# hkchengrex/Cutie

Measured on AMD Instinct MI355X. Metric: frames/sec (480p, 3 objects), higher is better.
Workload: dtype bf16

## Files before the change

cutie_amd/_lib.py:

```python
import ctypes
import os

_HERE = os.path.dirname(os.path.abspath(__file__))
LIB_PATH = os.environ.get('CUTIE_AMD_LIB') or os.path.join(_HERE, 'libcutie_hip.so')
ABI_VERSION = 11
OP_STRUCT_SIZE = 256

_lib = None


class HipLibraryError(RuntimeError):
    pass


def load():
    global _lib
    if _lib is not None:
        return _lib
    if not os.path.exists(LIB_PATH):
        raise HipLibraryError(
            f'{LIB_PATH} not found: build it with `python -c "import __graft_entry__ as g; g.build()"` '
            f'(or `make -C cutie_amd/csrc`).  cutie_amd has no CPU fallback.')
    lib = ctypes.CDLL(LIB_PATH)
    lib.cutie_exec.argtypes = [ctypes.c_void_p, ctypes.c_int, ctypes.c_void_p]
    lib.cutie_exec.restype = ctypes.c_int
    lib.cutie_exec_one.argtypes = [ctypes.c_void_p, ctypes.c_void_p]
    lib.cutie_exec_one.restype = ctypes.c_int
    lib.cutie_graph_capture.argtypes = [ctypes.c_void_p, ctypes.c_int, ctypes.c_void_p]
    lib.cutie_graph_capture.restype = ctypes.c_void_p
    lib.cutie_graph_launch.argtypes = [ctypes.c_void_p, ctypes.c_void_p]
    lib.cutie_graph_launch.restype = ctypes.c_int
    lib.cutie_graph_destroy.argtypes = [ctypes.c_void_p]
    lib.cutie_graph_destroy.restype = None
    lib.cutie_time_ops.argtypes = [ctypes.c_void_p, ctypes.c_int, ctypes.c_int, ctypes.c_void_p]
    lib.cutie_time_ops.restype = ctypes.c_float
    lib.cutie_hip_last_error.argtypes = []
    lib.cutie_hip_last_error.restype = ctypes.c_char_p
    lib.cutie_hip_abi_version.restype = ctypes.c_int
    lib.cutie_op_struct_size.restype = ctypes.c_int
    lib.cutie_hip_build_flags.restype = ctypes.c_int
    if lib.cutie_hip_abi_version() != ABI_VERSION or lib.cutie_op_struct_size() != OP_STRUCT_SIZE:
        raise HipLibraryError(f'{LIB_PATH} is stale (ABI {lib.cutie_hip_abi_version()}, '
                              f'op size {lib.cutie_op_struct_size()}); rebuild it.')
    _lib = lib
    return lib


EXPORTED_SYMBOLS = ['cutie_exec', 'cutie_exec_one', 'cutie_graph_capture', 'cutie_graph_launch',
                    'cutie_graph_destroy', 'cutie_time_ops', 'cutie_hip_last_error',
                    'cutie_hip_abi_version', 'cutie_op_struct_size', 'cutie_hip_build_flags']


def has_diag_kernels():
    return bool(load().cutie_hip_build_flags() & 1)


def has_png_decode():
    return bool(load().cutie_hip_build_flags() & 2)


def has_jpeg_batch():
    return bool(load().cutie_hip_build_flags() & 4)


def has_mixed_lockstep():
    return bool(load().cutie_hip_build_flags() & 8)


def has_track_stats():
    return bool(load().cutie_hip_build_flags() & 16)


class HipExecutor:
    is_mock = False

    def __init__(self):
        import torch
        self.lib = load()
        if not torch.cuda.is_available():
            raise HipLibraryError('no HIP device visible: cutie_amd runs on MI355X only (no CPU fallback).')
        self._torch = torch
        self._raw_stream = getattr(torch._C, '_cuda_getCurrentRawStream', None)
        self.graph_stats = [0, 0]
        self._warned = False

    def stream(self):
        raw = self._raw_stream
        if raw is not None:
            return raw(self._torch.cuda.current_device())
        return self._torch.cuda.current_stream().cuda_stream

    def run(self, arr):
        rc = self.lib.cutie_exec(arr.ctypes.data, len(arr), self.stream())
        if rc != 0:
            raise RuntimeError('cutie_exec failed: ' + self.lib.cutie_hip_last_error().decode())

    def run_on(self, arr, stream):
        rc = self.lib.cutie_exec(arr.ctypes.data, len(arr), stream.cuda_stream)
        if rc != 0:
            raise RuntimeError('cutie_exec failed: ' + self.lib.cutie_hip_last_error().decode())

    GRAPH_CACHE_ENTRIES = 24

    def run_cached(self, arr, cache, head=0):
        if head:
            self.run(arr[:head])
            arr = arr[head:]
        key = arr['p'].tobytes()
        ent = cache.get(key)
        if ent is None:
            if len(cache) >= self.GRAPH_CACHE_ENTRIES:
                old = cache.pop(next(iter(cache)))
                if old not in (0, -1):
                    self.lib.cutie_graph_destroy(old)
            cache[key] = 0
            self.graph_stats[0] += 1
            return self.run(arr)
        if ent == 0:
            ent = self.lib.cutie_graph_capture(arr.ctypes.data, len(arr), self.stream()) or -1
            cache[key] = ent
            if ent == -1 and not self._warned:
                self._warned = True
                import warnings
                warnings.warn('HIP graph capture of a launch plan failed (%s); such plans keep running launch by launch'
                              % self.lib.cutie_hip_last_error().decode())
        if ent == -1:
            self.graph_stats[0] += 1
            return self.run(arr)
        self.graph_stats[1] += 1
        if self.lib.cutie_graph_launch(ent, self.stream()) != 0:
            raise RuntimeError('cutie_graph_launch failed: ' + self.lib.cutie_hip_last_error().decode())

    def time_ops(self, arr, iters):
        ms = self.lib.cutie_time_ops(arr.ctypes.data, len(arr), iters, self.stream())
        if ms < 0:
            raise RuntimeError('cutie_time_ops failed: ' + self.lib.cutie_hip_last_error().decode())
        return ms


_executor = None


def get_executor():
    global _executor
    if _executor is None:
        _executor = HipExecutor()
    return _executor


def set_executor_for_testing(ex):
    global _executor
    _executor = ex
```

cutie_amd/csrc/api.hip:

```cpp
#include "common.h"
#include <stdarg.h>
#include <stdio.h>
#include <string.h>

static thread_local char g_err[512] = "";

void cutie_set_error(const char* fmt, ...) {
    va_list ap;
    va_start(ap, fmt);
    vsnprintf(g_err, sizeof(g_err), fmt, ap);
    va_end(ap);
}

static int dispatch(const cutie_op* op, hipStream_t s) {
    switch (op->kind) {
        case CUTIE_OP_CONV: return launch_conv(op, s);
        case CUTIE_OP_QUERY_INIT: return (op->flags & 1) ? launch_attention(op, s) : launch_elementwise(op, s);
        case CUTIE_OP_QFFN: return launch_qchain(op, s);
        case CUTIE_OP_STEM: return launch_stem(op, s);
        case CUTIE_OP_ATTN_Q2P: case CUTIE_OP_ATTN_SELF: case CUTIE_OP_ATTN_P2Q:
            return (op->flags & 12) ? launch_qchain(op, s) : launch_attention(op, s);
        case CUTIE_OP_AUX_MASK:
            return launch_attention(op, s);
        case CUTIE_OP_KEY_PREP: case CUTIE_OP_AFF_SCORE: case CUTIE_OP_AFF_SELECT: case CUTIE_OP_AFF_READOUT:
// ... 21 lines not shown
                cutie_set_error("op %d (kind %d): %s", k, ops[k].kind, tmp);
            }
            return rc > 0 ? -1 : rc;
        }
    }
    return 0;
}

int cutie_exec_one(const cutie_op* op, void* stream) { return cutie_exec(op, 1, stream); }

struct GraphHandle { hipGraph_t graph; hipGraphExec_t exec; };

void* cutie_graph_capture(const cutie_op* ops, int n, void* stream) {
    (void)stream;
    static thread_local hipStream_t cap = nullptr;
    if (!cap && hipStreamCreateWithFlags(&cap, hipStreamNonBlocking) != hipSuccess) {
        cap = nullptr;
        (void)hipGetLastError();
        cutie_set_error("graph: cannot create the capture stream");
        return nullptr;
    }
    hipGraph_t graph = nullptr;
    if (hipStreamBeginCapture(cap, hipStreamCaptureModeThreadLocal) != hipSuccess) {
        (void)hipGetLastError();
        cutie_set_error("graph: begin capture failed");
        return nullptr;
    }
    int rc = cutie_exec(ops, n, (void*)cap);
    hipError_t e = hipStreamEndCapture(cap, &graph);
    if (rc != 0 || e != hipSuccess || !graph) {
        if (graph) hipGraphDestroy(graph);
        if (rc == 0) cutie_set_error("graph: end capture failed (%d)", (int)e);
        (void)hipGetLastError();
        return nullptr;
    }
    hipGraphExec_t exec = nullptr;
    if (hipGraphInstantiate(&exec, graph, nullptr, nullptr, 0) != hipSuccess) {
        hipGraphDestroy(graph);
        (void)hipGetLastError();
        cutie_set_error("graph: instantiate failed");
        return nullptr;
    }
    GraphHandle* h = new GraphHandle{graph, exec};
    return h;
}

int cutie_graph_launch(void* graph, void* stream) {
    GraphHandle* h = (GraphHandle*)graph;
    if (!h) { cutie_set_error("graph: null handle"); return -4; }
    hipError_t e = hipGraphLaunch(h->exec, (hipStream_t)stream);
    if (e != hipSuccess) { cutie_set_error("graph launch: %s", hipGetErrorString(e)); return -1; }
    return 0;
}

void cutie_graph_destroy(void* graph) {
    GraphHandle* h = (GraphHandle*)graph;
    if (!h) return;
    hipGraphExecDestroy(h->exec);
    hipGraphDestroy(h->graph);
    delete h;
}

float cutie_time_ops(const cutie_op* ops, int n, int iters, void* stream) {
    hipStream_t s = (hipStream_t)stream;
    hipEvent_t a, b;
    if (hipEventCreate(&a) != hipSuccess || hipEventCreate(&b) != hipSuccess) { cutie_set_error("time: event create failed"); return -1.f; }
    if (cutie_exec(ops, n, stream) != 0) return -1.f;
    hipEventRecord(a, s);
    for (int it = 0; it < iters; ++it)
        if (cutie_exec(ops, n, stream) != 0) return -1.f;
    hipEventRecord(b, s);
    hipEventSynchronize(b);
    float ms = 0.f;
    hipEventElapsedTime(&ms, a, b);
    hipEventDestroy(a);
    hipEventDestroy(b);
    return ms / (float)iters;
}

const char* cutie_hip_last_error(void) { return g_err; }
int cutie_hip_abi_version(void) { return 11; }
int cutie_op_struct_size(void) { return (int)sizeof(cutie_op); }
int cutie_hip_build_flags(void) {
    const int forms = 2 | 4 | 8 | 16;
#ifdef CUTIE_DIAG
    return forms | 1;
#else
    return forms;
#endif
}

}
```

cutie_amd/csrc/elementwise.hip:

```cpp
#include "common.h"
#include <math.h>

#define GRID1D(n, bs) dim3((unsigned)(((long)(n) + (bs) - 1) / (bs)))
__global__ void memset32_kernel(uint32_t* d, long n, uint32_t v);

__global__ void maxpool_kernel(const uint4* __restrict__ x, uint4* __restrict__ y, int B, int H, int W, int C8,
                               int OH, int OW, int relu) {
    long idx = (long)blockIdx.x * blockDim.x + threadIdx.x;
    long total = (long)B * OH * OW * C8;
    if (idx >= total) return;
    int c = idx % C8; long t = idx / C8;
    int ow = t % OW; t /= OW; int oh = t % OH; int b = t / OH;
    float m[8];
#pragma unroll
    for (int i = 0; i < 8; ++i) m[i] = relu ? 0.f : -INFINITY;
    for (int dy = 0; dy < 3; ++dy) {
        int ih = oh * 2 - 1 + dy;
        if ((unsigned)ih >= (unsigned)H) continue;
        for (int dx = 0; dx < 3; ++dx) {
            int iw = ow * 2 - 1 + dx;
            if ((unsigned)iw >= (unsigned)W) continue;
            uint4 v = x[(((long)b * H + ih) * W + iw) * C8 + c];
            uint32_t u[4] = {v.x, v.y, v.z, v.w};
#pragma unroll
            for (int i = 0; i < 4; ++i) {
                m[2 * i] = fmaxf(m[2 * i], __uint_as_float(u[i] << 16));
                m[2 * i + 1] = fmaxf(m[2 * i + 1], __uint_as_float(u[i] & 0xffff0000u));
            }
        }
    }
    y[idx] = make_uint4(pack_bf2(m[0], m[1]), pack_bf2(m[2], m[3]), pack_bf2(m[4], m[5]), pack_bf2(m[6], m[7]));
}

__global__ void img_prep_kernel(const float* __restrict__ img, const float* __restrict__ masks, uint4* __restrict__ y,
                                int h0, int w0, int H, int W, int pl, int pt, int K,
                                float m0, float m1, float m2, float s0, float s1, float s2) {
    long idx = (long)blockIdx.x * blockDim.x + threadIdx.x;
    long HW = (long)H * W;
    if (idx >= HW * K) return;
    int k = idx / HW; long pix = idx - (long)k * HW;
    int yy = pix / W, xx = pix - (long)yy * W;
    int sy = yy - pt, sx = xx - pl;
    float r = 0.f, g = 0.f, b = 0.f;
    if ((unsigned)sy < (unsigned)h0 && (unsigned)sx < (unsigned)w0) {
        long o = (long)sy * w0 + sx, plane = (long)h0 * w0;
        r = img[o]; g = img[plane + o]; b = img[2 * plane + o];
    }
    r = (r - m0) / s0; g = (g - m1) / s1; b = (b - m2) / s2;
    float mk = 0.f, others = 0.f;
    if (masks) {
        float sum = 0.f;
        for (int j = 0; j < K; ++j) sum += masks[(long)j * HW + pix];
        mk = masks[(long)k * HW + pix];
        others = fminf(fmaxf(sum - mk, 0.f), 1.f);
    }
    y[idx] = make_uint4(pack_bf2(r, g), pack_bf2(b, mk), pack_bf2(others, 0.f), 0u);
}

__device__ __forceinline__ void up_coord(int o, int n_in, float scale, int& i0, int& i1, float& lam) {
    float src = ((float)o + 0.5f) * scale - 0.5f;
    if (src < 0.f) src = 0.f;
    i0 = (int)src;
    if (i0 > n_in - 1) i0 = n_in - 1;
    i1 = i0 + (i0 < n_in - 1 ? 1 : 0);
    lam = src - (float)i0;
}

template <bool MIXED = false>
__global__ void upsample2x_add_kernel(const uint4* __restrict__ g, const uint4* __restrict__ skip, uint4* __restrict__ y,
                                      int B, int h, int w, int C8, int Kg, long gstride, int prio) {
    if (prio) __builtin_amdgcn_s_setprio(1);
    long idx = (long)blockIdx.x * blockDim.x + threadIdx.x;
    int OH = 2 * h, OW = 2 * w;
    long total = (long)B * OH * OW * C8;
    if (idx >= total) return;
    int c = idx % C8; long t = idx / C8;
    int ox = t % OW; t /= OW; int oy = t % OH; int b = t / OH;
    int y0, y1, x0, x1; float ly, lx;
    up_coord(oy, h, 0.5f, y0, y1, ly);
    up_coord(ox, w, 0.5f, x0, x1, lx);
    const uint4* gb = g + (long)b * h * w * C8;
    uint4 v00 = gb[((long)y0 * w + x0) * C8 + c], v01 = gb[((long)y0 * w + x1) * C8 + c];
    uint4 v10 = gb[((long)y1 * w + x0) * C8 + c], v11 = gb[((long)y1 * w + x1) * C8 + c];
    long grp;
    if (MIXED) { int st; grp = mixed_clip_of((unsigned)Kg, b, st); }
    else grp = Kg > 0 ? b / Kg : 0;
    uint4 sk = skip[(grp * gstride + (long)oy * OW + ox) * C8 + c];
    const uint32_t* a = &v00.x; const uint32_t* bq = &v01.x; const uint32_t* cq = &v10.x; const uint32_t* d = &v11.x;
    const uint32_t* s = &sk.x;
    float w00 = (1.f - ly) * (1.f - lx), w01 = (1.f - ly) * lx, w10 = ly * (1.f - lx), w11 = ly * lx;
    uint32_t out[4];
#pragma unroll
    for (int i = 0; i < 4; ++i) {
        float lo = w00 * __uint_as_float(a[i] << 16) + w01 * __uint_as_float(bq[i] << 16) +
                   w10 * __uint_as_float(cq[i] << 16) + w11 * __uint_as_float(d[i] << 16) + __uint_as_float(s[i] << 16);
        float hi = w00 * __uint_as_float(a[i] & 0xffff0000u) + w01 * __uint_as_float(bq[i] & 0xffff0000u) +
                   w10 * __uint_as_float(cq[i] & 0xffff0000u) + w11 * __uint_as_float(d[i] & 0xffff0000u) +
                   __uint_as_float(s[i] & 0xffff0000u);
        out[i] = pack_bf2(lo, hi);
    }
    y[idx] = make_uint4(out[0], out[1], out[2], out[3]);
}

template <int R = 0>
__device__ __forceinline__ void area_down_bf16_body(const bf16_t* __restrict__ x, bf16_t* __restrict__ y, int B, int H, int W, int C,
                                                    int ldx, int ldy, int rrt, long idx) {
    const int r = R > 0 ? R : rrt;
    int C8 = C >> 3, OH = H / r, OW = W / r;
    long total = (long)B * OH * OW * C8;
    if (idx >= total) return;
    int c = idx % C8; long t = idx / C8;
    int ox = t % OW; t /= OW; int oy = t % OH; int b = t / OH;
    float acc[8] = {0, 0, 0, 0, 0, 0, 0, 0};
    if (R > 0) {
        uint4 v[R > 0 ? R * R : 1];
#pragma unroll
        for (int dy = 0; dy < R; ++dy)
#pragma unroll
            for (int dx = 0; dx < R; ++dx)
                v[dy * R + dx] = *reinterpret_cast<const uint4*>(x + (((long)b * H + oy * R + dy) * W + ox * R + dx) * ldx + c * 8);
#pragma unroll
        for (int e = 0; e < R * R; ++e) {
            const uint32_t* u = &v[e].x;
#pragma unroll
            for (int i = 0; i < 4; ++i) {
                acc[2 * i] += __uint_as_float(u[i] << 16);
                acc[2 * i + 1] += __uint_as_float(u[i] & 0xffff0000u);
            }
        }
    } else
    for (int dy = 0; dy < r; ++dy)
        for (int dx = 0; dx < r; ++dx) {
            const uint4 v = *reinterpret_cast<const uint4*>(x + (((long)b * H + oy * r + dy) * W + ox * r + dx) * ldx + c * 8);
            const uint32_t* u = &v.x;
#pragma unroll
            for (int i = 0; i < 4; ++i) {
                acc[2 * i] += __uint_as_float(u[i] << 16);
                acc[2 * i + 1] += __uint_as_float(u[i] & 0xffff0000u);
            }
        }
    float inv = 1.f / (float)(r * r);
    uint4 o = make_uint4(pack_bf2(acc[0] * inv, acc[1] * inv), pack_bf2(acc[2] * inv, acc[3] * inv),
                         pack_bf2(acc[4] * inv, acc[5] * inv), pack_bf2(acc[6] * inv, acc[7] * inv));
    *reinterpret_cast<uint4*>(y + (((long)b * OH + oy) * OW + ox) * ldy + c * 8) = o;
}
__global__ void area_down_bf16_kernel(const bf16_t* __restrict__ x, bf16_t* __restrict__ y, int B, int H, int W, int C,
                                      int ldx, int ldy, int r) {
    area_down_bf16_body(x, y, B, H, W, C, ldx, ldy, r, (long)blockIdx.x * blockDim.x + threadIdx.x);
}

template <int R = 0>
__device__ __forceinline__ void area_down_f32_body(const float* __restrict__ x, bf16_t* __restrict__ y, int B, int H, int W, int C,
                                                   int ldx, int ldy, int rrt, int Cz, long idx) {
    const int r = R > 0 ? R : rrt;
    int OH = H / r, OW = W / r;
    long total = (long)B * OH * OW;
    if (idx >= total) return;
    int ox = idx % OW; long t = idx / OW; int oy = t % OH; int b = t / OH;
    float inv = 1.f / (float)(r * r);
    bf16_t* yp = y + idx * ldy;
    for (int c = 0; c < C; ++c) {
        float acc = 0.f;
        if (R > 0) {
            float v[R > 0 ? R * R : 1];
#pragma unroll
            for (int dy = 0; dy < R; ++dy)
#pragma unroll
                for (int dx = 0; dx < R; ++dx) v[dy * R + dx] = x[(((long)b * H + oy * R + dy) * W + ox * R + dx) * ldx + c];
#pragma unroll
            for (int e = 0; e < R * R; ++e) acc += v[e];
        } else
        for (int dy = 0; dy < r; ++dy)
            for (int dx = 0; dx < r; ++dx) acc += x[(((long)b * H + oy * r + dy) * W + ox * r + dx) * ldx + c];
        yp[c] = f2bf(acc * inv);
    }
    for (int c = C; c < Cz; ++c) yp[c] = 0;
}
__global__ void area_down_f32_kernel(const float* __restrict__ x, bf16_t* __restrict__ y, int B, int H, int W, int C,
                                     int ldx, int ldy, int r, int Cz) {
    area_down_f32_body(x, y, B, H, W, C, ldx, ldy, r, Cz, (long)blockIdx.x * blockDim.x + threadIdx.x);
}
struct AreaSeg { const void* x; bf16_t* y; int B, H, W, C, ldx, ldy, r, Cz, f32; long n; };
struct Area3 { AreaSeg s[3]; int rt; int prio; };
__global__ void area_down3_kernel(Area3 a) {
// ... 57 lines not shown
            if (k0 + u >= K) break;
            const float a = wave_sum(acc[u]) / (float)(r * r);
            sum += a;
            if (lane == 0) m16[(long)(k0 + u) * hw + px] = a;
        }
    }
    if (lane == 0)
        for (int k = 0; k < K; ++k) {
            const float mk = m16[(long)k * hw + px];
            const float others = fminf(fmaxf(sum - mk, 0.f), 1.f);
            y[((long)k * hw + px) * ld8] = make_uint4(pack_bf2(mk, others), 0u, 0u, 0u);
        }
}
__global__ void mask_pair_kernel(const float* __restrict__ m16, uint4* __restrict__ y, int K, int hw) {
    long idx = (long)blockIdx.x * blockDim.x + threadIdx.x;
    if (idx >= (long)K * hw) return;
    int k = idx / hw; int p = idx - (long)k * hw;
    float sum = 0.f;
    for (int j = 0; j < K; ++j) sum += m16[(long)j * hw + p];
    float mk = m16[idx];
    float others = fminf(fmaxf(sum - mk, 0.f), 1.f);
    y[idx] = make_uint4(pack_bf2(mk, others), 0u, 0u, 0u);
}

__global__ __launch_bounds__(256) void gap_partial_kernel(const bf16_t* __restrict__ x, float* __restrict__ part, int HW, int C) {
    __shared__ float red[2048 + 32];
    const int b = blockIdx.y, p0 = blockIdx.x * 64;
    const int C8 = C >> 3;
    const int c8 = threadIdx.x % C8, rg = threadIdx.x / C8, nrg = 256 / C8;
    float acc[8] = {0, 0, 0, 0, 0, 0, 0, 0};
    for (int r = rg; r < 64; r += nrg) {
        int p = p0 + r;
        if (p < HW) {
            uint4 v = *reinterpret_cast<const uint4*>(x + ((long)b * HW + p) * C + c8 * 8);
            acc[0] += __uint_as_float(v.x << 16); acc[1] += __uint_as_float(v.x & 0xffff0000u);
            acc[2] += __uint_as_float(v.y << 16); acc[3] += __uint_as_float(v.y & 0xffff0000u);
            acc[4] += __uint_as_float(v.z << 16); acc[5] += __uint_as_float(v.z & 0xffff0000u);
            acc[6] += __uint_as_float(v.w << 16); acc[7] += __uint_as_float(v.w & 0xffff0000u);
        }
    }
#pragma unroll
    for (int i = 0; i < 8; ++i) red[rg * (C + 1) + c8 * 8 + i] = acc[i];
    __syncthreads();
    for (int c = threadIdx.x; c < C; c += 256) {
        float sum = 0.f;
        for (int g = 0; g < nrg; ++g) sum += red[g * (C + 1) + c];
        part[((long)b * gridDim.x + blockIdx.x) * C + c] = sum;
    }
}
__global__ void gap_final_kernel(const float* __restrict__ part, float* __restrict__ y, int nchunk, int C, float inv) {
    const int b = blockIdx.x;
    for (int c = threadIdx.x; c < C; c += blockDim.x) {
        float sum = 0.f;
        for (int k = 0; k < nchunk; ++k) sum += part[((long)b * nchunk + k) * C + c];
        y[(long)b * C + c] = sum * inv;
    }
}

__global__ __launch_bounds__(256) void eca_apply_kernel(const bf16_t* __restrict__ x, const float* __restrict__ part,
                                                        const float* __restrict__ wk, const bf16_t* __restrict__ r,
                                                        bf16_t* __restrict__ y, float* __restrict__ gap_out, int HW, int C, int nchunk,
                                                        const long long* __restrict__ fixed, const bf16_t* __restrict__ pw,
                                                        const float* __restrict__ pb, float* __restrict__ plog, int prio) {
    if (prio) __builtin_amdgcn_s_setprio(1);
    __shared__ float gap[256 + 4], sc[256];
    const int b = blockIdx.y, tid = threadIdx.x;
    const float inv = 1.f / (float)HW;
    const int C8 = C >> 3;
    const int p0 = blockIdx.x * 32;
    uint4 xv[4], rv[4];
    long offs[4];
#pragma unroll
    for (int it = 0; it < 4; ++it) {
        const int q = tid + it * 256;
        const int pp = q / C8, c8 = q - pp * C8, p = p0 + pp;
        const bool ok = q < 32 * C8 && p < HW;
        offs[it] = ok ? ((long)b * HW + p) * C + c8 * 8 : -1;
        const long o = ok ? offs[it] : 0;
        xv[it] = *reinterpret_cast<const uint4*>(x + o);
        rv[it] = *reinterpret_cast<const uint4*>(r + o);
    }
    if (fixed) {
        for (int c = tid; c < C; c += 256) {
            const float mean = (float)((double)fixed[(long)b * C + c] * (1.0 / 16777216.0)) * inv;
            gap[c + 2] = mean;
            if (gap_out && blockIdx.x == 0) gap_out[(long)b * C + c] = mean;
        }
    } else
    for (int c = tid; c < C; c += 256) {
        float sum = 0.f;
        for (int k0 = 0; k0 < nchunk; k0 += 8) {
            float v[8];
#pragma unroll
            for (int u = 0; u < 8; ++u) v[u] = part[((long)b * nchunk + min(k0 + u, nchunk - 1)) * C + c];
#pragma unroll
            for (int u = 0; u < 8; ++u) sum += k0 + u < nchunk ? v[u] : 0.f;
        }
        gap[c + 2] = sum * inv;
        if (gap_out && blockIdx.x == 0) gap_out[(long)b * C + c] = sum * inv;
    }
    if (tid < 2) { gap[tid] = 0.f; gap[C + 2 + tid] = 0.f; }
    __syncthreads();
    for (int c = tid; c < C; c += 256) {
        float a = wk[0] * gap[c] + wk[1] * gap[c + 1] + wk[2] * gap[c + 2] + wk[3] * gap[c + 3] + wk[4] * gap[c + 4];
        sc[(c & 7) * 32 + (c >> 3)] = sigmoidf_(a);
    }
    __syncthreads();
#pragma unroll
    for (int it = 0; it < 4; ++it) {
        if (offs[it] < 0) continue;
        const int q = tid + it * 256;
        const int c8 = q % C8;
        const uint32_t* xu = &xv[it].x; const uint32_t* ru = &rv[it].x;
        uint32_t o[4];
#pragma unroll
        for (int i = 0; i < 4; ++i) {
            float lo = __uint_as_float(xu[i] << 16) * sc[(2 * i) * 32 + c8] + __uint_as_float(ru[i] << 16);
            float hi = __uint_as_float(xu[i] & 0xffff0000u) * sc[(2 * i + 1) * 32 + c8] + __uint_as_float(ru[i] & 0xffff0000u);
            o[i] = pack_bf2(lo, hi);
        }
        *reinterpret_cast<uint4*>(y + offs[it]) = make_uint4(o[0], o[1], o[2], o[3]);
    }
    if (pw) {
        const int c8 = tid & 31;
        const uint4 wv = *reinterpret_cast<const uint4*>(pw + c8 * 8);
        const uint32_t* wu = &wv.x;
        const float bias = pb ? pb[0] : 0.f;
#pragma unroll
        for (int it = 0; it < 4; ++it) {
            float part = 0.f;
            if (offs[it] >= 0) {
                const uint32_t* xu = &xv[it].x; const uint32_t* ru = &rv[it].x;
#pragma unroll
                for (int i = 0; i < 4; ++i) {
                    const float lo = __uint_as_float(xu[i] << 16) * sc[(2 * i) * 32 + c8] + __uint_as_float(ru[i] << 16);
                    const float hi = __uint_as_float(xu[i] & 0xffff0000u) * sc[(2 * i + 1) * 32 + c8] + __uint_as_float(ru[i] & 0xffff0000u);
                    const uint32_t st = pack_bf2(lo, hi);
                    part += fmaxf(__uint_as_float(st << 16), 0.f) * __uint_as_float(wu[i] << 16);
                    part += fmaxf(__uint_as_float(st & 0xffff0000u), 0.f) * __uint_as_float(wu[i] & 0xffff0000u);
                }
            }
            part += __uint_as_float(__builtin_amdgcn_update_dpp(0, (int)__float_as_uint(part), 0xB1, 0xf, 0xf, false));
            part += __uint_as_float(__builtin_amdgcn_update_dpp(0, (int)__float_as_uint(part), 0x4E, 0xf, 0xf, false));
            part += __uint_as_float(__builtin_amdgcn_update_dpp(0, (int)__float_as_uint(part), 0x141, 0xf, 0xf, false));
            part += __uint_as_float(__builtin_amdgcn_update_dpp(0, (int)__float_as_uint(part), 0x140, 0xf, 0xf, false));
            const unsigned pu = __float_as_uint(part);
            const auto rr = __builtin_amdgcn_permlane16_swap(pu, pu, false, false);
            const float tot = __uint_as_float(rr[0]) + __uint_as_float(rr[1]);
            const int q = tid + it * 256, p = p0 + q / C8;
            if (c8 == 0 && offs[it] >= 0) plog[(long)b * HW + p] = tot + bias;
        }
    }
}

__global__ void gru4_kernel(const float* __restrict__ v, float* __restrict__ h, bf16_t* __restrict__ hb, long n, int C, int prio) {
    if (prio) __builtin_amdgcn_s_setprio(1);
    const long idx = (long)blockIdx.x * blockDim.x + threadIdx.x;
    const int C4 = C >> 2;
    if (idx >= n * C4) return;
    const long row = idx / C4; const int c = (int)(idx - row * C4) * 4;
    const float* vr = v + row * 3 * C + c;
    const float4 f4 = *reinterpret_cast<const float4*>(vr), u4 = *reinterpret_cast<const float4*>(vr + C), n4 = *reinterpret_cast<const float4*>(vr + 2 * C);
    const float4 h4 = *reinterpret_cast<const float4*>(h + row * C + c);
    const float fa[4] = {f4.x, f4.y, f4.z, f4.w}, ua[4] = {u4.x, u4.y, u4.z, u4.w}, na[4] = {n4.x, n4.y, n4.z, n4.w}, ha[4] = {h4.x, h4.y, h4.z, h4.w};
    float o[4];
#pragma unroll
    for (int i = 0; i < 4; ++i) {
        const float f = sigmoidf_(fa[i]), u = sigmoidf_(ua[i]), nv = tanhf(na[i]);
        o[i] = f * ha[i] * (1.f - u) + u * nv;
    }
    *reinterpret_cast<float4*>(h + row * C + c) = make_float4(o[0], o[1], o[2], o[3]);
    *reinterpret_cast<uint2*>(hb + row * C + c) = make_uint2(pack_bf2(o[0], o[1]), pack_bf2(o[2], o[3]));
}

__global__ void gru_kernel(const float* __restrict__ v, float* __restrict__ h, bf16_t* __restrict__ hb, long n, int C) {
    long idx = (long)blockIdx.x * blockDim.x + threadIdx.x;
    if (idx >= n * C) return;
    long row = idx / C; int c = idx - row * C;
    const float* vr = v + row * 3 * C;
    float f = sigmoidf_(vr[c]), u = sigmoidf_(vr[C + c]), nv = tanhf(vr[2 * C + c]);
    float nh = f * h[idx] * (1.f - u) + u * nv;
    h[idx] = nh;
    hb[idx] = f2bf(nh);
}

__device__ __forceinline__ float clamp_logit(float p) {
    p = fminf(fmaxf(p, 1e-7f), 1.f - 1e-7f);
    return logf(p / (1.f - p));
}

__global__ void seg_agg_kernel(const float* __restrict__ lg, float* __restrict__ agg, int K, int hw) {
    int p = blockIdx.x * blockDim.x + threadIdx.x;
    if (p >= hw) return;
    float bg = 1.f;
    for (int k = 0; k < K; ++k) {
        float pr = 1.f / (1.f + expf(-lg[(long)k * hw + p]));
        bg *= (1.f - pr);
        agg[(long)(k + 1) * hw + p] = clamp_logit(pr);
    }
    agg[p] = clamp_logit(bg);
}

__global__ void up4_softmax_kernel(const float* __restrict__ agg, float* __restrict__ prob, float* __restrict__ lup,
                                   int P, int h, int w) {
    int OH = 4 * h, OW = 4 * w;
    long idx = (long)blockIdx.x * blockDim.x + threadIdx.x;
    if (idx >= (long)OH * OW) return;
    int ox = idx % OW, oy = idx / OW;
    int y0, y1, x0, x1; float ly, lx;
    up_coord(oy, h, 0.25f, y0, y1, ly);
    up_coord(ox, w, 0.25f, x0, x1, lx);
    float w00 = (1.f - ly) * (1.f - lx), w01 = (1.f - ly) * lx, w10 = ly * (1.f - lx), w11 = ly * lx;
    long o00 = (long)y0 * w + x0, o01 = (long)y0 * w + x1, o10 = (long)y1 * w + x0, o11 = (long)y1 * w + x1;
    long hw = (long)h * w, OHW = (long)OH * OW;
    float mx = -INFINITY;
    for (int c = 0; c < P; ++c) {
        const float* a = agg + c * hw;
        float v = w00 * a[o00] + w01 * a[o01] + w10 * a[o10] + w11 * a[o11];
        if (lup) lup[c * OHW + idx] = v;
        mx = fmaxf(mx, v);
    }
    float sum = 0.f;
    for (int c = 0; c < P; ++c) {
        const float* a = agg + c * hw;
        float v = w00 * a[o00] + w01 * a[o01] + w10 * a[o10] + w11 * a[o11];
        sum += expf(v - mx);
    }
    float inv = 1.f / sum;
    for (int c = 0; c < P; ++c) {
        const float* a = agg + c * hw;
        float v = w00 * a[o00] + w01 * a[o01] + w10 * a[o10] + w11 * a[o11];
// ... 807 lines not shown
#pragma unroll
    for (int k = 0; k < 4; ++k)
        if (ox0 + k < OW) o[k] = (OUT)lut[arg[k]];
}

template <typename OUT>
__global__ void prob_to_id_merge_kernel(const uint64_t* __restrict__ srcs, const int4* __restrict__ geom, const int* __restrict__ lut,
                                        OUT* __restrict__ out, int S, int P, int OH, int OW, int packed) {
    const int OW4 = (OW + 3) >> 2;
    const long idx = (long)blockIdx.x * blockDim.x + threadIdx.x;
    if (idx >= (long)OH * OW4) return;
    const int oy = (int)(idx / OW4), ox0 = (int)(idx - (long)oy * OW4) * 4;
    int best[4], arg[4];
#pragma unroll
    for (int k = 0; k < 4; ++k) { best[k] = 0; arg[k] = 0; }
    for (int q = 0; q < P; ++q) {
        int sum[4] = {0, 0, 0, 0};
        for (int sI = 0; sI < S; ++sI) {
            const int4 g = geom[sI];
            const int H = g.x, W = g.y;
            if (H < 1 || W < 1) continue;
            const float* prob = (const float*)srcs[sI] + (long)q * g.z;
            const float sy = (float)H / (float)OH, sx = (float)W / (float)OW;
            const float fy = fmaxf((oy + 0.5f) * sy - 0.5f, 0.f);
            const int y0 = min((int)fy, H - 1), y1 = min(y0 + 1, H - 1);
            const float ly = fy - (float)y0;
            const float* r0 = prob + (long)y0 * g.w;
            const float* r1 = prob + (long)y1 * g.w;
#pragma unroll
            for (int k = 0; k < 4; ++k) {
                const int ox = min(ox0 + k, OW - 1);
                const float fx = fmaxf((ox + 0.5f) * sx - 0.5f, 0.f);
                const int x0 = min((int)fx, W - 1), x1 = min(x0 + 1, W - 1);
                const float lx = fx - (float)x0;
                const float a = r0[x0], b = r0[x1], cc = r1[x0], d = r1[x1];
                const float v = (1.f - ly) * ((1.f - lx) * a + lx * b) + ly * ((1.f - lx) * cc + lx * d);
                sum[k] += (int)(uint8_t)(int)(v * 255.f);
            }
        }
#pragma unroll
        for (int k = 0; k < 4; ++k)
            if (q == 0 || sum[k] > best[k]) { best[k] = sum[k]; arg[k] = q; }
    }
    OUT* o = out + (long)oy * OW + ox0;
    if constexpr (sizeof(OUT) == 1) {
        if (packed) {
            *(uint32_t*)o = (uint32_t)(uint8_t)lut[arg[0]] | (uint32_t)(uint8_t)lut[arg[1]] << 8 | (uint32_t)(uint8_t)lut[arg[2]] << 16 |
                            (uint32_t)(uint8_t)lut[arg[3]] << 24;
            return;
        }
    } else {
        if (packed) {
            *(int4*)o = make_int4(lut[arg[0]], lut[arg[1]], lut[arg[2]], lut[arg[3]]);
            return;
        }
    }
#pragma unroll
    for (int k = 0; k < 4; ++k)
        if (ox0 + k < OW) o[k] = (OUT)lut[arg[k]];
}

int launch_elementwise(const cutie_op* op, hipStream_t s) {
    const int32_t* i = op->i;
    const uint64_t* p = op->p;
    const int BS = 256;
    const int PRIO = (op->flags & CUTIE_F_PRIO) ? 1 : 0;
    switch (op->kind) {
        case CUTIE_OP_MAXPOOL: {
            int C8 = i[3] / 8;
            long n = (long)i[0] * i[4] * i[5] * C8;
            hipLaunchKernelGGL(maxpool_kernel, GRID1D(n, BS), dim3(BS), 0, s, (const uint4*)p[0], (uint4*)p[1], i[0], i[1], i[2], C8, i[4], i[5], op->flags & 1);
            break;
        }
        case CUTIE_OP_IMG_PREP: {
            int K = p[1] ? i[6] : 1;
            long n = (long)i[2] * i[3] * K;
            hipLaunchKernelGGL(img_prep_kernel, GRID1D(n, BS), dim3(BS), 0, s, (const float*)p[0], (const float*)p[1], (uint4*)p[2],
                               i[0], i[1], i[2], i[3], i[4], i[5], K, op->f[0], op->f[1], op->f[2], op->f[3], op->f[4], op->f[5]);
            break;
        }
        case CUTIE_OP_UPSAMPLE2X_ADD: {
            int C8 = i[3] / 8;
            long n = (long)i[0] * 4 * i[1] * i[2] * C8;
            if (i[6]) {
                int objs; const int nc = mixed_clips((unsigned)i[6], &objs);
                if (nc < 1 || objs != i[0] || i[4] != 0 || i[5] < 4 * i[1] * i[2]) { cutie_set_error("upsample2x_add (mixed form): the counts 0x%x do not add up to B = %d (or i4 != 0, or the stride is below one map)", i[6], i[0]); return -2; }
                hipLaunchKernelGGL(upsample2x_add_kernel<true>, GRID1D(n, BS), dim3(BS), 0, s, (const uint4*)p[0], (const uint4*)p[1], (uint4*)p[2], i[0], i[1], i[2], C8, i[6], (long)i[5], PRIO);
                break;
            }
            if (i[4] < 0 || (i[4] > 0 && (i[0] % i[4] || i[5] < 4 * i[1] * i[2]))) { cutie_set_error("upsample2x_add: skip groups of %d objects do not divide B = %d (or their stride is below one map)", i[4], i[0]); return -2; }
            hipLaunchKernelGGL(upsample2x_add_kernel<false>, GRID1D(n, BS), dim3(BS), 0, s, (const uint4*)p[0], (const uint4*)p[1], (uint4*)p[2], i[0], i[1], i[2], C8, i[4], (long)i[5], PRIO);
            break;
        }
        case CUTIE_OP_AREA_DOWN: {
            int r = i[6];
            long np = (long)i[0] * (i[1] / r) * (i[2] / r);
            if (op->flags & 1)
                hipLaunchKernelGGL(area_down_f32_kernel, GRID1D(np, BS), dim3(BS), 0, s, (const float*)p[0], (bf16_t*)p[1], i[0], i[1], i[2], i[3], i[4], i[5], r, i[7]);
            else
                hipLaunchKernelGGL(area_down_bf16_kernel, GRID1D(np * (i[3] / 8), BS), dim3(BS), 0, s, (const bf16_t*)p[0], (bf16_t*)p[1], i[0], i[1], i[2], i[3], i[4], i[5], r);
            break;
        }
        case CUTIE_OP_AREA_DOWN3: {
            Area3 a;
            long total = 0;
            for (int q = 0; q < 3; ++q) {
                const int32_t* j = i + 8 * q;
                AreaSeg& g = a.s[q];
                g.x = (const void*)p[2 * q]; g.y = (bf16_t*)p[2 * q + 1];
                g.B = j[0]; g.H = j[1]; g.W = j[2]; g.C = j[3]; g.ldx = j[4]; g.ldy = j[5]; g.r = j[6]; g.Cz = j[7];
                g.f32 = (op->flags >> q) & 1;
                if (g.r < 1 || (!g.f32 && (g.C & 7))) { cutie_set_error("area_down3: segment %d: r >= 1, C %% 8 for bf16 input", q); return -2; }
                const long np = (long)g.B * (g.H / g.r) * (g.W / g.r);
                g.n = g.f32 ? np : np * (g.C / 8);
                total += g.n;
            }
            a.rt = (op->flags >> 3) & 1;
            a.prio = PRIO;
            hipLaunchKernelGGL(area_down3_kernel, GRID1D(total, BS), dim3(BS), 0, s, a);
            break;
        }
        case CUTIE_OP_MASK_DOWN: {
            int K = i[0], r = i[3], h = i[1] / r, w = i[2] / r;
            long n = (long)K * h * w;
            float* m16 = (float*)p[2];
            if (!m16) { cutie_set_error("mask_down: m16 buffer required"); return -2; }
            hipLaunchKernelGGL(mask_down_pair_kernel, GRID1D((long)h * w * 64, BS), dim3(BS), 0, s, (const float*)p[0], m16, (uint4*)p[1], K, i[1], i[2], r,
                               i[4] > 8 ? i[4] / 8 : 1);
            break;
        }
        case CUTIE_OP_GAP: {
            if (i[2] > 256 || (i[2] & 7) || 256 % (i[2] / 8)) { cutie_set_error("gap: C must divide 256 octet-wise (C=%d)", i[2]); return -2; }
            if (!p[2]) { cutie_set_error("gap: scratch buffer required"); return -2; }
            int nchunk = (i[1] + 63) / 64;
            hipLaunchKernelGGL(gap_partial_kernel, dim3(nchunk, i[0]), dim3(256), 0, s, (const bf16_t*)p[0], (float*)p[2], i[1], i[2]);
            if (!(op->flags & 1))
                hipLaunchKernelGGL(gap_final_kernel, dim3(i[0]), dim3(256), 0, s, (const float*)p[2], (float*)p[1], nchunk, i[2], 1.f / (float)i[1]);
            break;
        }
        case CUTIE_OP_ECA_APPLY: {
            if (i[2] > 256 || (i[2] & 7)) { cutie_set_error("eca: C <= 256, C %% 8"); return -2; }
            if (p[6] && (i[2] != 256 || !p[8])) { cutie_set_error("eca: the fused 1x1 head needs C = 256 and an output"); return -2; }
            int nchunk = (i[1] + 63) / 64;
            hipLaunchKernelGGL(eca_apply_kernel, dim3((i[1] + 31) / 32, i[0]), dim3(256), 0, s, (const bf16_t*)p[0], (const float*)p[5], (const float*)p[2],
                               (const bf16_t*)p[3], (bf16_t*)p[4], (float*)p[1], i[1], i[2], nchunk, (op->flags & 1) ? (const long long*)p[5] : nullptr,
                               (const bf16_t*)p[6], (const float*)p[7], (float*)p[8], PRIO);
            break;
        }
        case CUTIE_OP_GRU: {
            long n = (long)i[0] * i[1];
            if (!(op->flags & 1) && (i[1] & 3) == 0 && (((uintptr_t)p[0] | (uintptr_t)p[1]) & 15) == 0 && ((uintptr_t)p[2] & 7) == 0)
                hipLaunchKernelGGL(gru4_kernel, GRID1D(n / 4, BS), dim3(BS), 0, s, (const float*)p[0], (float*)p[1], (bf16_t*)p[2], (long)i[0], i[1], PRIO);
            else
                hipLaunchKernelGGL(gru_kernel, GRID1D(n, BS), dim3(BS), 0, s, (const float*)p[0], (float*)p[1], (bf16_t*)p[2], (long)i[0], i[1]);
            break;
        }
        case CUTIE_OP_SEG_AGG:
            hipLaunchKernelGGL(seg_agg_kernel, GRID1D(i[1], BS), dim3(BS), 0, s, (const float*)p[0], (float*)p[1], i[0], i[1]);
            break;
        case CUTIE_OP_UP4_SOFTMAX: {
            long n = (long)16 * i[1] * i[2];
            if (op->flags & 1) {
                if (i[0] > 16) { cutie_set_error("up4_softmax: the fused form holds P <= 16 planes in registers (P=%d)", i[0]); return -2; }
                const bool vec = !(op->flags & 2) && i[0] <= 8 && (((uintptr_t)p[1] | (uintptr_t)p[2]) & 15) == 0;
                const int nclip = i[4] > 1 ? i[4] : 1;
                if (nclip > 1 && !vec) { cutie_set_error("up4_softmax: several clips per launch need the four-pixel form (P <= 8, aligned outputs)"); return -2; }
// ... 235 lines not shown
```

cutie_amd/inference/inference_core.py:

```python
import contextlib
import logging
import os
from typing import List, Optional

import numpy as np
import torch

from .. import _lib, frame_context, ops as O
from ..model import plans
from .image_feature_store import ImageFeatureStore
from .memory_manager import MemoryManager
from .object_manager import ObjectManager

log = logging.getLogger()
F32 = torch.float32
DEFER_MEM = os.environ.get('CUTIE_AMD_DEFER_MEM', '0') not in ('', '0')
WAIT_TRACE = None
AFF_BATCH = int(os.environ.get('CUTIE_AMD_AFF_BATCH', '8'))
AFF_FIRST_ALONE = os.environ.get('CUTIE_AMD_AFF_FIRST_ALONE', '1') not in ('', '0')
WINDOW = int(os.environ.get('CUTIE_AMD_WINDOW', '12'))
WINDOW_LEAD = int(os.environ.get('CUTIE_AMD_WINDOW_LEAD', '3'))


def pad_geometry(h, w, d=16):
# ... 296 lines not shown
        if out is None:
            out = torch.empty_like(x)
        W = x.shape[-1]
        ol = O.OpList()
        ol.flip_w(x, out, rows=x.numel() // W, W=W, alpha=alpha, beta=beta)
        ol.finalize()
        ol.run()
        return out

    def clear_memory(self):
        self._join_pending()
        self.curr_ti = -1
        self.last_mem_ti = 0
        ovf = self.memory._scratch.get('overflow')
        self.memory._join_side()
        self.memory = MemoryManager(cfg=self.cfg, object_manager=self.object_manager)
        if ovf is not None:
            self.memory._scratch['overflow'] = ovf
        if self._prefetched is not None:
            if self._prefetched[3] is not None:
                torch.cuda.current_stream(self._prefetched[1].device).wait_event(self._prefetched[3])
            self._prefetched = self._prefetched_rec = self._prefetched_group = None
        if self._flip is not None:
            self._flip.clear_memory()

    def clear_non_permanent_memory(self):
        self._join_pending()
        self.curr_ti = -1
        self.last_mem_ti = 0
        self.memory.clear_non_permanent_memory()
        if self._flip is not None:
            self._flip.clear_non_permanent_memory()

    def clear_sensory_memory(self):
        self._join_pending()
        self.curr_ti = -1
        self.last_mem_ti = 0
        self.memory.clear_sensory_memory()
        if self._flip is not None:
            self._flip.clear_sensory_memory()

    def update_config(self, cfg):
        self._join_pending()
        self.mem_every = cfg['mem_every']
        self.memory.update_config(cfg)
        if self._flip is not None:
            self._flip.update_config(cfg)

    def _add_memory(self, image, pix_feat, prob, key, shrinkage, selection, *, is_deep_update=True, force_permanent=False):
        if prob.shape[1] == 0:
            log.warning('Trying to add an empty object mask to memory!')
            return
        as_permanent = 'all' if force_permanent else 'first'
        ids = self.object_manager.all_obj_ids
        self.memory.initialize_sensory_if_needed(key, ids)
        g = frame_context.recall('geometry', image)
        raw = (image, g[0], g[1], g[4], g[5]) if g is not None else None
        pre = self._prefetched
        if (pre is not None and self._prefetched_rec is not None and self._flip is None
                and self._lane_of_other is None):
            msk_value, finish = self.network.encode_mask(
                image, pix_feat, self.memory.get_sensory(ids), prob, deep_update=is_deep_update, chunk_size=self.chunk_size,
                need_weights=self.save_aux, _raw=raw, _split=True)
            self.memory.add_memory(key, shrinkage, msk_value, None, ids, selection=selection, as_permanent=as_permanent)
            feats = pre[2]
            ev = self._ahead_affinity(feats[2], feats[4], pre[3], self._prefetched_rec, next_mem_ti=self.curr_ti + self.mem_every, first_alone=AFF_FIRST_ALONE)
            self._prefetched = pre[:3] + (ev,) + pre[4:]
            sensory, obj_value = finish()
            self.memory.add_object_values(obj_value, ids)
        else:
            msk_value, sensory, obj_value, _ = self.network.encode_mask(
                image, pix_feat, self.memory.get_sensory(ids), prob, deep_update=is_deep_update, chunk_size=self.chunk_size,
                need_weights=self.save_aux, _raw=raw)
            self.memory.add_memory(key, shrinkage, msk_value, obj_value, ids, selection=selection, as_permanent=as_permanent)
        self.last_mem_ti = self.curr_ti
        if is_deep_update:
            self.memory.update_sensory(sensory, ids)

    def _segment(self, key, selection, pix_feat, ms_features, update_sensory=True) -> torch.Tensor:
        if not self.memory.engaged:
            log.warning('Trying to segment without any memory!')
            return torch.zeros((1, key.shape[-2] * 16, key.shape[-1] * 16), device=key.device, dtype=key.dtype)
        ids = self.object_manager.all_obj_ids
        memory_readout = self.memory.read(pix_feat, key, selection, self.last_mask, self.network)
        stacked = self.memory.readout_stacked(ids)
        memory_readout = stacked if stacked is not None else self.object_manager.realize_dict(memory_readout)
        sensory, _, pred_prob_with_bg = self.network.segment(ms_features, memory_readout, self.memory.get_sensory(ids),
                                                             chunk_size=self.chunk_size, update_sensory=update_sensory,
                                                             _need_logits=False, _fork=self._hinted)
        pred_prob_with_bg = pred_prob_with_bg[0]
        if update_sensory:
            self.memory.update_sensory(sensory, ids)
        return pred_prob_with_bg

    def step(self, image: torch.Tensor, mask: Optional[torch.Tensor] = None, objects: Optional[List[int]] = None, *,
             idx_mask: bool = True, end: bool = False, delete_buffer: bool = True, force_permanent: bool = False,
             next_image: Optional[torch.Tensor] = None, next_images=None) -> torch.Tensor:
        if objects is None and mask is not None:
            assert not idx_mask
            objects = list(range(1, mask.shape[0] + 1))

        resize_needed = False
        if self.max_internal_size > 0:
            h, w = image.shape[-2:]
            min_side = min(h, w)
            if min_side > self.max_internal_size:
                resize_needed = True
                new_h = int(h / min_side * self.max_internal_size)
                new_w = int(w / min_side * self.max_internal_size)
                image = self._resize(image, (new_h, new_w))
                if mask is not None:
                    if idx_mask:
                        mask = self._resize(mask.unsqueeze(0).float(), (new_h, new_w), nearest=True)[0].round().long()
                    else:
                        mask = self._resize(mask, (new_h, new_w))

        self.curr_ti += 1
        if self._lane_of_other is None:
            self.network.engine().pool.tick()
        pre, self._prefetched, self._prefetched_rec = self._prefetched, None, None
        self._prefetched_group = None
        if self._window and not resize_needed and (pre is None or pre[0] != self._frame_key(image)):
            ent = self._window.get(self._frame_key(image))
            if ent is not None:
                if pre is not None and pre[3] is not None:
                    torch.cuda.current_stream(pre[1].device).wait_event(pre[3])
                pre = (self._frame_key(image), ent[0], self.network._adopt_encoded(ent[1]), ent[2], ent[3], ent[4])
        if pre is not None and not resize_needed and pre[0] == self._frame_key(image):
            image = pre[1]
            if pre[3] is not None:
                if WAIT_TRACE is not None:
                    a, b = torch.cuda.Event(enable_timing=True), torch.cuda.Event(enable_timing=True)
                    a.record()
                    torch.cuda.current_stream(image.device).wait_event(pre[3])
                    b.record()
                    WAIT_TRACE.append((self.curr_ti, a, b))
                else:
                    torch.cuda.current_stream(image.device).wait_event(pre[3])
            self.image_feature_store._store[self.curr_ti] = pre[2]
            self._window.pop(pre[0], None)
            h0, w0, H, W, pl, pt = pre[5]
            frame_context.remember('geometry', image, pre[5])
            self.pad = pad_geometry(h0, w0, 16)[2]
        else:
            if pre is not None and pre[3] is not None:
                torch.cuda.current_stream(pre[1].device).wait_event(pre[3])
            image, (h0, w0, H, W, self.pad) = self._prepare_image(image)
            pl, pt = self.pad[0], self.pad[2]

        self._hinted = (next_image is not None or (next_images is not None and len(next_images) > 0)) and self._flip is None
        is_mem_frame = ((self.curr_ti - self.last_mem_ti >= self.mem_every) or (mask is not None)) and (not end)
        need_segment = (mask is None) or (self.object_manager.num_obj > 0 and not self.object_manager.has_all(objects))
        update_sensory = ((self.curr_ti - self.last_mem_ti) in self.stagger_ti) and (not end)

        ms_feat, pix_feat = self.image_feature_store.get_features(self.curr_ti, image)
        key, shrinkage, selection = self.image_feature_store.get_key(self.curr_ti, image)
        self._join_pending()
        fl = self._flip
        if fl is not None:
            fl.curr_ti, fl.pad = self.curr_ti, self.pad
            image_f = self._flip_w(image)
            frame_context.remember('geometry', image_f, (h0, w0, H, W, self.pad[1], pt))
            ms_f, pix_f = fl.image_feature_store.get_features(self.curr_ti, image_f)
            key_f, shr_f, sel_f = fl.image_feature_store.get_key(self.curr_ti, image_f)
        elif (next_image is not None or (next_images is not None and len(next_images) > 0)) and not end:
            aff = not (is_mem_frame or force_permanent) and self.memory.engaged
            if next_images is not None and len(next_images) > 0:
                self.prefetch_window(next_images, affinity=aff)
# ... 126 lines not shown
```

cutie_amd/inference/lockstep.py:

```python
import contextlib
import os
from typing import List, Optional, Sequence

import torch

from .. import _lib, frame_context
from .. import ops as O
from ..model import plans
from ..model.cutie import group_logical
from . import inference_core as IC
from .inference_core import InferenceCore, pad_geometry, unpad

BF16, F32 = torch.bfloat16, torch.float32


class ClipCores:

    def __init__(self, network, cfg, n: int):
        self.cores = [InferenceCore(network, cfg) for _ in range(n)]
        for c, core in enumerate(self.cores):
            core.memory._clip_tag = c
        self._ctx = [frame_context.new_context() for _ in range(n)]

    @contextlib.contextmanager
# ... 265 lines not shown
                t0, t = r0[name], r[name]
                if t.data_ptr() != t0.data_ptr() + c * ws * t0[0].numel() * t0.element_size():
                    return False
        return True

    def step(self, images: Sequence[torch.Tensor], masks: Optional[Sequence] = None, objects: Optional[Sequence] = None, *,
             end: bool = False, next_images: Optional[Sequence[Sequence[torch.Tensor]]] = None, **kw) -> List[torch.Tensor]:
        cores = self.cores
        assert len(images) == len(cores)
        if not self._batchable(images, masks, end):
            self._drop_lookahead()
            self._md_valid = False
            out = []
            for c, core in enumerate(cores):
                with frame_context.context(self._ctx[c]):
                    out.append(core.step(images[c], None if masks is None else masks[c], None if objects is None else objects[c], end=end, **kw))
            return out
        assert not kw, 'a lock-step frame takes images and look-ahead hints only'
        return self._step_batched(images, next_images)

    def _step_batched(self, images, next_images):
        cores, net = self.cores, self.network
        eng = net.engine()
        dev = net.device
        gpu = dev.type == 'cuda'
        G = len(cores)
        for c, core in enumerate(cores):
            core.curr_ti += 1
            core.memory._clip_tag = c
        eng.pool.tick()
        keys = [core._frame_key(img) for core, img in zip(cores, images)]
        ent = [core._window.pop(k, None) for core, k in zip(cores, keys)]
        if not self._one_batch(ent):
            for core, k, e in zip(cores, keys, ent):
                if e is not None:
                    core._window[k] = e
            self._drop_lookahead()
            self._encode_batch([[img] for img in images], [[k] for k in keys], ahead=False)
            ent = [core._window.pop(k) for core, k in zip(cores, keys)]
        if gpu and ent[0][2] is not None:
            torch.cuda.current_stream(dev).wait_event(ent[0][2])
        recs = [e[1] for e in ent]
        prepared = [e[0] for e in ent]
        h0, w0, H, W, pl, pt = ent[0][4]
        feats = []
        for c, core in enumerate(cores):
            core.pad = pad_geometry(h0, w0, 16)[2]
            core._prefetched = core._prefetched_rec = None
            with frame_context.context(self._ctx[c]):
                feats.append(net._adopt_encoded(recs[c]))
        c0 = cores[0]
        is_mem_frame = c0.curr_ti - c0.last_mem_ti >= c0.mem_every
        update_sensory = (c0.curr_ti - c0.last_mem_ti) in c0.stagger_ti
        counts, st, mixed = self._counts()
        K = counts[0]
        lay = (counts, 0) if mixed else (G, K)
        clips = counts if mixed else G
        sf, sb, ov = self._stack_state(counts, st)
        if next_images is not None and len(next_images) == G:
            self._prefetch(next_images, affinity=not is_mem_frame)
        h, w = recs[0]['h'], recs[0]['w']
        readouts = []
        stacked = recs[0]['_qo'].pop('_readouts_joint', None)
        for c, core in enumerate(cores):
            with frame_context.context(self._ctx[c]):
                vis = core.memory.read_visual(recs[c]['_qo'], h, w, dev, net)
            readouts.append(next(iter(vis.values())))
        if stacked is not None and any(r.data_ptr() != stacked[c * K].data_ptr() or r.shape[0] != K for c, r in enumerate(readouts)):
            stacked = None
        self.stacked_steps += stacked is not None
        ws = recs[0]['_wstride']
        m = net.model_cfg
        KT = st[-1]
        md = self._md_valid
        P = eng.plan(('ls_fuse',) + lay + (h, w, md, ws, stacked is not None), plans.build_pixel_fusion, K, h, w, True, md, clips, ws, stacked is not None)
        fused = eng.pool.get(('ls_fuse',) + lay + (h, w, eng.devstr), dict(fused=((KT, h, w, m['embed_dim']), BF16, False)), dev)['fused']
        dyn = {'pixel%d' % c: readouts[c] for c in range(G)} if stacked is None else dict(pixel=stacked)
        if not md:
            dyn.update({'last_mask%d' % c: _f32c(core.last_mask[0]) for c, core in enumerate(cores)})
        P.run(sensory_bf16=sb, fuse_xt=recs[0]['fuse_xt'], fused=fused, **dyn)
        token = tuple(core.memory._objv_token for core in cores)
        fresh = token != self._qtoken or not plans.QINIT_SKIP
        self._qtoken = token
        P = eng.plan(('ls_rq',) + lay + (h, w, fresh), plans.build_readout_query, K, h, w, False, fresh, clips)
        out = eng.pool.get(('ls_rq',) + lay + (h, w, eng.devstr), dict(out=((KT, h, w, m['embed_dim']), BF16, False)), dev)['out']
        P.run(pixel=fused, obj_mem=ov, out=out)
        P = eng.plan(('ls_seg',) + lay + (h, w, bool(update_sensory), ws), plans.build_segment, K, h, w, bool(update_sensory), True, True, clips, ws)
        prob = eng.pool.get(('ls_seg',) + lay + (h, w, eng.devstr), dict(prob=((KT + G, 16 * h, 16 * w) if mixed else (G, K + 1, 16 * h, 16 * w), F32, False)), dev)['prob']
        P.run(p16=out, sensory_f32=sf, sensory_bf16=sb, prob=prob, logits_up=None, f8p=recs[0]['f8p'], f4p=recs[0]['f4p'])
        self._md_valid = True
        probs = [prob[st[c] + c:st[c + 1] + c + 1] for c in range(G)] if mixed else [prob[c] for c in range(G)]
        for c, core in enumerate(cores):
            core.last_mask = probs[c][1:].unsqueeze(0)
        if is_mem_frame:
            self._memorise(prepared, recs, feats, prob, (h0, w0, H, W, pl, pt), (counts, st, mixed), next_images)
        self.batched_steps += 1
        return [unpad(probs[c], core.pad) for c, core in enumerate(cores)]

    def _memorise(self, prepared, recs, feats, prob, geometry, layout, next_images):
        cores, net = self.cores, self.network
        eng = net.engine()
        dev = net.device
        G = len(cores)
        h0, w0, H, W, pl, pt = geometry
        h, w = H // 16, W // 16
        m = net.model_cfg
        sf, sb, _ = self._state
        ws = recs[0]['_wstride']
        counts, st, mixed = layout
        K, KT = counts[0], st[-1]
        lay = (counts, 0) if mixed else (G, K)
        md = self._md_valid
        P = eng.plan(('ls_emask',) + lay + (h0, w0, H, W, pl, pt, md, ws), plans.build_encode_mask, K, h0, w0, H, W, pl, pt, True, md, counts if mixed else G, ws)
        o = eng.pool.get(('ls_emask',) + lay + (h, w, eng.devstr),
                         dict(value=((KT, h, w, m['value_dim']), BF16, False),
                              summ=((KT, m['object_summarizer']['num_summaries'], m['embed_dim'] + 1), F32, False)), dev)
        value, summ = o['value'], o['summ']
        dyn = dict(masks=prob, pix_feat=recs[0]['pix_feat'], sensory_f32=sf, sensory_bf16=sb, value=value, summ=summ,
                   **{'image%d' % c: prepared[c] for c in range(G)})
        cut = P.meta['value_done']
        P.run_part(0, cut, **dyn)
        for c, core in enumerate(cores):
            ids = core.object_manager.all_obj_ids
            _, _, key, shrinkage, selection = feats[c]
            with frame_context.context(self._ctx[c]):
                core.memory.add_memory(key, shrinkage, group_logical(value[st[c]:st[c + 1]]), None, ids, selection=selection, as_permanent='first')
        if next_images is not None:
            nxt = []
            for c, core in enumerate(cores):
                grp = core._prefetched_group
                ent = core._window.get(grp[1][0]) if grp is not None and len(grp[1]) else None
                if ent is not None:
                    with frame_context.context(self._ctx[c]):
                        f = net._adopt_encoded(ent[1])
                    nxt.append((c, core, ent, f))
            joint = len(nxt) == G and self._ahead_joint(cores[0].curr_ti + cores[0].mem_every, first_alone=IC.AFF_FIRST_ALONE)
            for part in (() if joint else ('first', 'rest') if IC.AFF_FIRST_ALONE else (None,)):
                for c, core, ent, f in nxt:
                    with frame_context.context(self._ctx[c]):
                        core._ahead_affinity(f[2], f[4], ent[2], ent[1], next_mem_ti=core.curr_ti + core.mem_every,
                                             first_alone=IC.AFF_FIRST_ALONE, part=part)
        P.run_part(cut, None, first=False, **dyn)
        for c, core in enumerate(cores):
            ids = core.object_manager.all_obj_ids
            with frame_context.context(self._ctx[c]):
                core.memory.add_object_values(summ[st[c]:st[c + 1]].unsqueeze(0), ids)
            core.last_mem_ti = core.curr_ti

    def output_prob_to_mask(self, probs: Sequence[torch.Tensor], **kw) -> List[torch.Tensor]:
        return [core.output_prob_to_mask(p, **kw) for core, p in zip(self.cores, probs)]

    def __getitem__(self, c: int) -> InferenceCore:
        return self.cores[c]

    def delete_objects(self, objects: Sequence[Sequence[int]]) -> None:
        for c, (core, ids) in enumerate(zip(self.cores, objects)):
            if ids:
                with frame_context.context(self._ctx[c]):
                    core.delete_objects(list(ids))

    def _each(self, method, *a, **k):
        self._drop_lookahead()
        self._md_valid = False
        for c, core in enumerate(self.cores):
            with frame_context.context(self._ctx[c]):
                getattr(core, method)(*a, **k)

    def clear_memory(self):
        self._each('clear_memory')

    def clear_non_permanent_memory(self):
        self._each('clear_non_permanent_memory')
# ... 13 lines not shown
```

cutie_amd/inference/memory_manager.py:

```python
import itertools
import logging
import os
from typing import Dict, List

import torch

from .. import frame_context, ops as O
from .kv_memory_store import Bucket, StoreView, LIFE_EPS_BITS
from .object_manager import ObjectManager

log = logging.getLogger()
BF16, F32 = torch.bfloat16, torch.float32
CAND_CAP = 1024
_VALIDATE = os.environ.get('CUTIE_AMD_VALIDATE', '0') not in ('', '0')
PATCH_PLANS = os.environ.get('CUTIE_AMD_PATCH_PLANS', '1') not in ('', '0')
_VERSIONS = itertools.count(1)


class MemoryManager:
    def __init__(self, cfg, object_manager: ObjectManager):
        self.object_manager = object_manager
        self.sensory_dim = cfg.model.sensory_dim
        self.top_k = cfg.top_k
        self.chunk_size = cfg.chunk_size
# ... 347 lines not shown
        pool = network.engine().pool
        gbuf = m0._buf_rows('gmax_tau#joint', rows * Gld + rows, (), F32, dev)
        gmax, tau = gbuf[:rows * Gld], gbuf[rows * Gld:]
        cval = m0._buf_rows('cand_val#joint', rows, (CAND_CAP,), F32, dev)
        cidx = m0._buf_rows('cand_idx#joint', rows, (CAND_CAP,), torch.int32, dev)
        count = m0._buf_rows('count#joint', rows, (O.OpList.AFF_CSTRIDE,), torch.int32, dev)
        ovf = m0._buf('overflow', (1,), torch.int32, dev)
        spec = dict(r=((E, K, h, w, m0.CV), BF16, False))
        readout = pool.get_ring(('readout#joint', C, E, K, h, w, str(dev)), spec, dev, ring=3)['r']
        nslots = sig(b0)[2]
        clear_long = m0.use_long_term and b0.n_long > 0 and not m0.count_long_term_usage
        flat = [v for r in ranges for v in r] + [0] * (6 - 2 * len(ranges))
        key = (len(ranges), K, HW, HWp, m0.top_k, m0.use_long_term, clear_long, nslots, E, C)
        vals = (tuple(flat), G, b0.n_long)
        plans_ = m0.__dict__.setdefault('_joint_plans', {})
        cached = plans_.get((E, prio))
        if cached is not None and cached[0] == key:
            if cached[1] != vals:
                ol, ops_ = cached[2], cached[3]
                for op in (ops_['score0'], ops_['score1']):
                    ol.patch_ints(op, 3, flat + [G])
                ol.patch_ints(ops_['select'], 2, [G])
                for op in ops_['clear']:
                    ol.patch_ints(op, 0, [2 * b0.n_long])
                plans_[(E, prio)] = cached = (key, vals, ol, ops_)
        else:
            D = O.Dyn
            ol = O.OpList()
            ops_ = dict(clear=[])
            common = dict(HW=HW, HWp=HWp, ranges=ranges, cap=CAND_CAP, frames=E, nq=2, banks=(D('table'), C), prio=prio)
            ops_['score0'] = ol.aff_score(None, None, None, D('Bhi'), D('Blo'), D('cq'), D('gmax'), None, None, None, mode=0, **common)
            ops_['select'] = ol.aff_select(D('gmax'), D('tau'), HW=HW, HWp=HWp, G=G, top_k=m0.top_k, clear_count=D('count'), frames=E,
                                           zero=(D('usage'), 2 * E * nslots) if m0.use_long_term else None, prio=prio)
            ops_['score1'] = ol.aff_score(None, None, None, D('Bhi'), D('Blo'), D('cq'), D('tau'), D('cval'), D('cidx'), D('count'),
                                          mode=1, gmax_precedes_tau=True, **common)
            ol.aff_readout(D('cval'), D('cidx'), D('count'), D('vptrs'), D('usage') if m0.use_long_term else None, D('readout'),
                           D('ovf'), HW=HW, cap=CAND_CAP, top_k=m0.top_k, K=K, CV=m0.CV, frames=E, HWp=HWp, usage_stride=nslots, banks=C, prio=prio, usage_fx=True)
            if clear_long:
                for e in range(E):
                    ops_['clear'].append(ol.memset32(D('usage', 8 * e * nslots), 2 * b0.n_long, 0))
            plans_[(E, prio)] = cached = (key, vals, ol, ops_)
        ptrs = tuple((b.Ahi.data_ptr(), b.Alo.data_ptr(), b.scale.data_ptr(), b.vptrs().data_ptr()) for b in bs)
        tbl = m0.__dict__.get('_joint_table')
        if tbl is None or tbl[0] != ptrs:
            table = torch.tensor([list(p[:3]) for p in ptrs], dtype=torch.int64).to(dev)
            tbl = m0._joint_table = (ptrs, table, torch.cat([b.vptrs() for b in bs]), [b.vptrs() for b in bs])
        dyn = dict(count=count, table=tbl[1], Bhi=q0['Bhi'], Blo=q0['Blo'], cq=q0['cq'], gmax=gmax, tau=tau, cval=cval, cidx=cidx,
                   vptrs=tbl[2], readout=readout, ovf=ovf)
        udelta = None
        if m0.use_long_term:
            m0._joint_parity = m0.__dict__.get('_joint_parity', 0) ^ 1
            udelta = m0._buf_rows(f'udelta#joint{m0._joint_parity}', E, (nslots,), torch.int64, dev)
            dyn.update(usage=udelta)
        cached[2].run(**dyn)
        ev = event_factory() if event_factory is not None else None
        for e, q in enumerate(qs):
            mm, b = mms[e % C], bs[e % C]
            q['_readouts'] = {b.id: (readout[e], mm._version, udelta[e] if udelta is not None else None)}
            q['_readouts_ev'] = ev
            if e % C == 0:
                q['_readouts_joint'] = readout[e:e + C].view(C * K, h, w, m0.CV)
        return True

    def read_visual(self, q: dict, h: int, w: int, dev, network) -> Dict[int, torch.Tensor]:
        self._pool = network.engine().pool
        ahead = q.pop('_readouts', None) or {}
        ahead_ev = q.pop('_readouts_ev', None)
        if ahead_ev is not None and ahead:
            torch.cuda.current_stream(dev).wait_event(ahead_ev)
        out = {}
        for bucket in self.buckets.values():
            K = len(bucket.objects)
            pre = ahead.get(bucket.id)
            if pre is not None and pre[1] == self._version and pre[0].shape[0] == K:
                out[bucket.id] = pre[0]
                if pre[2] is not None:
                    self._commit_ahead(bucket, pre[2], network)
            else:
                self._join_side()
                out[bucket.id] = self._affinity(bucket, q, h, w, dev)
        return out

    def read(self, pix_feat: torch.Tensor, query_key: torch.Tensor, selection: torch.Tensor, last_mask: torch.Tensor,
             network) -> Dict[int, torch.Tensor]:
        q = network.query_operands(query_key, selection)
        h, w = pix_feat.shape[-2:]
        dev = pix_feat.device
        visual = self.read_visual(q, h, w, dev, network)
        all_readout = {}
        for bucket in self.buckets.values():
            K = len(bucket.objects)
            readout = visual[bucket.id]
            cs = self.chunk_size if (self.chunk_size is not None and self.chunk_size >= 1) else K
            chunks = []
            for c0 in range(0, K, cs):
                objects = bucket.objects[c0:c0 + cs]
                this_sensory = self.get_sensory(objects)
                this_last_mask = self._get_mask_by_ids(last_mask, objects)
                visual_readout = readout[c0:c0 + cs].permute(0, 3, 1, 2).unsqueeze(0)
                pixel_readout = network.pixel_fusion(pix_feat, visual_readout, this_sensory, this_last_mask)
                a, b = self._rows(objects, self._objv_ids)
                this_obj_mem = self._objv[a:b].unsqueeze(0).unsqueeze(2)
                readout_memory, aux_features = network.readout_query(pixel_readout, this_obj_mem, _last_aux=self.save_aux,
                                                                     _summary_token=(self._objv_token, a, b))
                for i, obj in enumerate(objects):
                    all_readout[obj] = readout_memory[:, i]
                chunks.append((objects, readout_memory))
                if self.save_aux:
                    self.aux = self._aux_output(this_sensory, pixel_readout, aux_features, Q=int(this_obj_mem.shape[3]))
            self._last_readout = chunks[0] if len(chunks) == 1 else (None, None)
        if _VALIDATE:
            self.check_overflow()
        return all_readout

    @staticmethod
    def _aux_output(sensory, pixel_readout, aux_features, Q: int = 16) -> dict:
        logits = [t.float().clone() for t in aux_features['logits']] if aux_features else None
        attn_mask = None
        if logits:
            lg = logits[-1]
            prob = torch.sigmoid(lg)
            bg = torch.prod(1 - prob, dim=1, keepdim=True).clamp(1e-7, 1 - 1e-7)
            pr = prob.clamp(1e-7, 1 - 1e-7)
            agg = torch.cat([torch.log(bg / (1 - bg)), torch.log(pr / (1 - pr))], 1)
            fg = agg[:, 1:] >= agg.max(dim=1, keepdim=True)[0]
            m = torch.cat([(~fg).unsqueeze(2).expand(-1, -1, Q // 2, -1, -1), fg.unsqueeze(2).expand(-1, -1, Q // 2, -1, -1)], 2).clone()
            full = m.flatten(3).all(-1)
            m[full] = False
            attn_mask = m.float()
        return {'sensory': sensory, 'pixel_readout': pixel_readout, 'q_logits': logits, 'q_weights': None, 'p_weights': None,
                'attn_mask': attn_mask}

    def check_overflow(self) -> int:
        ovf = self._scratch.get('overflow')
        if ovf is None:
            return 0
        n = int(ovf.item())
        if n:
            log.warning(f'affinity read-out: {n} queries had more than {CAND_CAP} candidates above the top-k threshold; '
                        f'their read-out used a truncated candidate list')
            ovf.zero_()
        return n

    def readout_stacked(self, all_obj_ids):
        objs, t = getattr(self, '_last_readout', (None, None))
        if objs is not None and list(objs) == list(all_obj_ids):
            return t
        return None

    def add_memory(self, key, shrinkage, msk_value, obj_value, objects: List[int], selection=None, *, as_permanent=False) -> None:
        assert as_permanent in ['no', 'first', 'all']
        self._join_side()
        self._version = next(_VERSIONS)
        bs = key.shape[0]
        assert bs == 1 and shrinkage.shape[0] == 1 and msk_value.shape[0] == 1
        self.engaged = True
        if self.H is None or self.config_stale:
            self.config_stale = False
            self.H, self.W = msk_value.shape[-2:]
            self.HW = self.H * self.W
            self.max_work_tokens = self.max_mem_frames * self.HW
            if self.use_long_term:
                self.min_work_tokens = self.min_mem_frames * self.HW
            for b in self.buckets.values():
                self._fit_bucket(b)
        HW = self.HW
        dev = key.device
        self.CK = key.shape[1]
        self.CV = msk_value.shape[2]
        kphys = key[0].permute(1, 2, 0).reshape(HW, self.CK)
        sphys = shrinkage.reshape(HW)
        ephys = selection[0].permute(1, 2, 0).reshape(HW, self.CK) if selection is not None else None
        kphys, sphys = kphys.to(F32).contiguous(), sphys.to(F32).contiguous()
        if ephys is not None:
            ephys = ephys.to(F32).contiguous()
        vphys = msk_value[0].permute(0, 2, 3, 1)
        if vphys.dtype != BF16 or not vphys.is_contiguous():
            vphys = vphys.to(BF16).contiguous()
        vphys = vphys.reshape(len(objects), HW, self.CV)

        ol = O.OpList()
        if obj_value is not None:
            self.add_object_values(obj_value, objects, ol)

        enabled = []
        new_objs = [o for o in objects if not any(o in b.objects for b in self.buckets.values())]
        if new_objs:
# ... 186 lines not shown
```

cutie_amd/model/cutie.py:

```python
import logging
from typing import Dict, Iterable, List

import torch
import torch.nn as nn

from .. import _lib, frame_context
from . import plans
from .param_spec import build_spec
from .weights import fold_bn, pack_conv, pack_linear, linear_as_conv

log = logging.getLogger()
BF16, F32 = torch.bfloat16, torch.float32


def nhwc_of(t, C=None):
    p = t.permute(0, 2, 3, 1)
    if p.dtype != BF16 or not p.is_contiguous():
        p = p.to(BF16).contiguous()
    return p


def group_nhwc_of(t, dtype=BF16):
    assert t.shape[0] == 1, 'batch size 1 only (flip_aug is not supported yet)'
    p = t[0].permute(0, 2, 3, 1)
# ... 90 lines not shown
            self._pe_wb[b] = wpe.float()
            we_ = sd[t + '.pixel_emb_proj.weight'].float().reshape(C, -1)
            W[q + '.pixel_proj_x'] = pack_conv(torch.cat([wm.float(), wpe.float() @ we_], 1).reshape(3 * C, 2 * C, 1, 1),
                                               bm.float() + wpe.float() @ sd[t + '.pixel_emb_proj.bias'].float(), dev, segs=[(C, C), (C, C)])
            W[q + '.read_from_pixel.q'] = pack_linear(Wp[:C], bp[:C], dev)
            W[q + '.read_from_pixel.out'] = pack_linear(sd[rp + '.out_proj.weight'], sd[rp + '.out_proj.bias'], dev)
            W[q + '.self_attn.qkv'] = pack_linear(Ws, bs, dev)
            W[q + '.self_attn.out'] = pack_linear(sd[sa + '.out_proj.weight'], sd[sa + '.out_proj.bias'], dev)
            W[q + '.read_from_query.kv'] = pack_linear(Wq[C:], bq[C:], dev)
            W[q + '.read_from_query.out'] = linear_as_conv(sd[rq + '.out_proj.weight'], sd[rq + '.out_proj.bias'], dev)
            for ln in ('.read_from_pixel.norm', '.self_attn.norm', '.ffn.norm'):
                W[q + ln + '.weight'] = sd[q + ln + '.weight'].to(dev).contiguous()
                W[q + ln + '.bias'] = sd[q + ln + '.bias'].to(dev).contiguous()
            W[q + '.ffn.linear1'] = pack_linear(sd[q + '.ffn.linear1.weight'], sd[q + '.ffn.linear1.bias'], dev)
            W[q + '.ffn.linear2'] = pack_linear(sd[q + '.ffn.linear2.weight'], sd[q + '.ffn.linear2.bias'], dev)
        conv(t + '.pixel_init_proj')
        for b in range(ot['num_blocks'] + 1):
            conv(f'{t}.mask_pred.{b}.1')
        for name in ca_blocks:
            conv(name + '.conv1')
            conv(name + '.conv2')
            W[name + '.conv.weight'] = sd[name + '.conv.weight'].reshape(-1).to(dev).contiguous()
        W[t + '.summary_to_query_init'] = pack_linear(sd[t + '.summary_to_query_init.weight'], sd[t + '.summary_to_query_init.bias'], dev)
        W[t + '.summary_to_query_emb'] = pack_linear(sd[t + '.summary_to_query_emb.weight'], sd[t + '.summary_to_query_emb.bias'], dev)
        u = 'object_summarizer'
        w_in, b_in = sd[u + '.input_proj.weight'].float(), sd[u + '.input_proj.bias'].float()
        w0 = torch.cat([sd[u + '.feature_pred.0.weight'].float(), sd[u + '.weights_pred.0.weight'].float()], 0)
        b0 = torch.cat([sd[u + '.feature_pred.0.bias'].float(), sd[u + '.weights_pred.0.bias'].float()], 0)
        self._sum_w0 = w0
        W[u + '.in_fw0'] = linear_as_conv(w0 @ w_in, b0 + w0 @ b_in, dev)
        wf2, ww2 = sd[u + '.feature_pred.2.weight'].float(), sd[u + '.weights_pred.2.weight'].float()
        cf, cw = wf2.shape[1], ww2.shape[1]
        w2 = torch.zeros(wf2.shape[0] + ww2.shape[0], cf + cw)
        w2[:wf2.shape[0], :cf] = wf2
        w2[wf2.shape[0]:, cf:] = ww2
        W[u + '.fw2'] = linear_as_conv(w2, torch.cat([sd[u + '.feature_pred.2.bias'].float(), sd[u + '.weights_pred.2.bias'].float()], 0), dev)

    def pe_rb(self, h, w, b):
        key = ('pe_rb', h, w, b)
        if key not in self._pe:
            e = plans.positional_encoding(h, w, self.m['embed_dim'], self.m['pixel_pe_scale'], self.m['pixel_pe_temperature'])
            e = e.reshape(h * w, -1).float()
            self._pe[key] = (e @ self._pe_wb[b].t()).to(BF16).to(self.device).contiguous()
        return self._pe[key]

    def pe_sum(self, h, w):
        key = ('pe_sum', h, w)
        if key not in self._pe:
            e = plans.positional_encoding(h, w, self.m['embed_dim'], self.m['pixel_pe_scale'], self.m['pixel_pe_temperature'])
            self._pe[key] = (e.reshape(h * w, -1).float() @ self._sum_w0.t()).to(BF16).to(self.device).contiguous()
        return self._pe[key]

    def rep_embedding(self, which, K):
        key = (which, K)
        if key not in self._rep:
            e = self.sd[f'object_transformer.{which}.weight']
            self._rep[key] = e.repeat(K, 1).to(self.device).contiguous()
        return self._rep[key]

    def mask_down_bufs(self, K, h, w, clips=1):
        mb = self.__dict__.setdefault('_md_bufs', {})
        if (K, h, w, clips) not in mb:
            mb[(K, h, w, clips)] = (torch.zeros((K, h, w, 64), dtype=BF16, device=self.device), torch.zeros((K, h, w), dtype=F32, device=self.device))
        return mb[(K, h, w, clips)]

    def query_bufs(self, K):
        qb = self.__dict__.setdefault('_query_bufs', {})
        if K not in qb:
            M = K * self.m['object_transformer']['num_queries']
            qb[K] = tuple(torch.zeros((M, self.m['embed_dim']), dtype=F32, device=self.device) for _ in range(2))
        return qb[K]

    def fork(self):
        e = object.__new__(Engine)
        e.__dict__.update(self.__dict__)
        e._plans = {}
        e._arenas = {}
        e.pool = plans.SlotPool()
        e.__dict__.pop('_splitk_part', None)
        e.__dict__.pop('_streams', None)
        e.__dict__.pop('_query_bufs', None)
        e.__dict__.pop('_md_bufs', None)
        e.__dict__.pop('_qinit_state', None)
        return e

    def plan(self, key, builder, *args):
        p = self._plans.get(key)
        if p is None:
            p = builder(self, *args)
            p.ol.finalize()
            kind = 'side' if key[0] in ('enc', 'key') else ('win' if key[0] == 'encw' else 'main')
            arenas = self.__dict__.setdefault('_arenas', {})
            if kind not in arenas:
                arenas[kind] = plans.Arena(self.device)
            p.pack_into(arenas[kind])
            self._plans[key] = p
        return p


class _Container(nn.Module):
    pass


class CUTIE(nn.Module):
    def __init__(self, cfg, *, single_object=False):
        super().__init__()
        if single_object:
            raise NotImplementedError('single_object=True is a training-time variant; not on the inference path')
        self.cfg = cfg
        m = cfg.model if hasattr(cfg, 'model') else cfg['model']
        self.model_cfg = m
        self.ms_dims = m['pixel_encoder']['ms_dims']
        self.key_dim, self.value_dim = m['key_dim'], m['value_dim']
        self.sensory_dim, self.pixel_dim, self.embed_dim = m['sensory_dim'], m['pixel_dim'], m['embed_dim']
        self.single_object = single_object
        self.object_transformer_enabled = m['object_transformer']['num_blocks'] > 0
        if not self.object_transformer_enabled:
            raise NotImplementedError('num_blocks == 0 is not supported')
        self._spec = build_spec(m)
        g = torch.Generator().manual_seed(0)
        for name, (shape, role) in self._spec.items():
            self._register(name, shape, role, g)
        self.register_buffer('pixel_mean', torch.tensor(m['pixel_mean'], dtype=F32).view(-1, 1, 1), False)
        self.register_buffer('pixel_std', torch.tensor(m['pixel_std'], dtype=F32).view(-1, 1, 1), False)
        self._eng = None
        self._key_cache = None
        self.eval()

    def _register(self, name, shape, role, g):
        parts = name.split('.')
        mod = self
        for p in parts[:-1]:
            if not hasattr(mod, p):
                mod.add_module(p, _Container())
            mod = getattr(mod, p)
        leaf = parts[-1]
        if role in ('w', 'emb', 'eca'):
            fan_in = max(1, int(torch.tensor(shape[1:]).prod())) if len(shape) > 1 else 1
            t = torch.randn(shape, generator=g) * (1.0 / fan_in ** 0.5)
            mod.register_parameter(leaf, nn.Parameter(t))
        elif role in ('b', 'bn_b', 'ln_b'):
            mod.register_parameter(leaf, nn.Parameter(torch.zeros(shape)))
        elif role in ('bn_w', 'ln_w'):
            mod.register_parameter(leaf, nn.Parameter(torch.ones(shape)))
        elif role == 'bn_mean':
            mod.register_buffer(leaf, torch.zeros(shape))
        elif role == 'bn_var':
            mod.register_buffer(leaf, torch.ones(shape))
        elif role == 'bn_nbt':
            mod.register_buffer(leaf, torch.tensor(0, dtype=torch.long))
        elif role == 'buf':
            dim = shape[0] * 2
            inv = 1.0 / (self.model_cfg['pixel_pe_temperature'] ** (torch.arange(0, dim, 2).float() / dim))
            mod.register_buffer(leaf, inv)
        else:
            raise KeyError(role)

    def train(self, mode=True):
        return super().train(False)

    def _apply(self, fn, *a, **k):
        self._eng = None
        return super()._apply(fn, *a, **k)

    def load_state_dict(self, *a, **k):
        self._eng = None
# ... 158 lines not shown
            qo = o['_qo'] = dict(Bhi=o['Bhi'], Blo=o['Blo'], cq=o['cq'], h=o['h'], w=o['w'])
        frame_context.remember('query', o['key'], qo, cap=4)
        return key, (shr if need_sk else None), (sel if need_ek else None)

    def query_operands(self, query_key: torch.Tensor, selection: torch.Tensor) -> dict:
        o = frame_context.recall('query', query_key)
        if o is not None:
            return o
        assert query_key.dim() == 4 and query_key.shape[0] == 1 and selection is not None, 'query key [1,CK,h,w] with its selection'
        h, w = query_key.shape[-2:]
        hw, HWp = h * w, -(-h * w // 64) * 64
        dev = self.device
        kphys = query_key[0].permute(1, 2, 0).reshape(hw, -1).to(device=dev, dtype=F32).contiguous()
        ephys = selection[0].permute(1, 2, 0).reshape(hw, -1).to(device=dev, dtype=F32).contiguous()
        o = dict(key=kphys, sel=ephys, Bhi=torch.zeros((HWp, 128), dtype=BF16, device=dev), Blo=torch.zeros((HWp, 128), dtype=BF16, device=dev),
                 cq=torch.zeros((HWp,), dtype=F32, device=dev), h=h, w=w)
        from .. import ops as O
        ol = O.OpList()
        ol.key_prep(kphys, ephys, o['Bhi'], o['Blo'], o['cq'], n=hw, query=True)
        ol.run()
        frame_context.remember('query', query_key, o, cap=4)
        return o

    @staticmethod
    def _sensory_pair(sensory):
        phys = group_nhwc_of(sensory, F32)
        shadow = frame_context.recall('sensory_bf16', phys)
        if shadow is None or shadow.shape != phys.shape:
            shadow = phys.to(BF16)
        return phys, shadow

    def encode_mask(self, image, ms_features, sensory, masks, *, deep_update=True, chunk_size=-1, need_weights=False,
                    _raw=None, _split=False):
        eng = self.engine()
        dev = eng.device
        K = masks.shape[1]
        H, W = masks.shape[-2:]
        h, w = H // 16, W // 16
        if _raw is not None:
            img, h0, w0, pl, pt = _raw
        else:
            img, h0, w0, pl, pt = image[0], H, W, 0, 0
        pix = nhwc_of(ms_features)
        sf, sb = self._sensory_pair(sensory)
        mk = f32c(masks[0])
        md = frame_context.recall('mask_down', mk)
        md = md is not None and md == (K, h, w, eng.__dict__.get('_md_gen'))
        P = eng.plan(('emask', K, h0, w0, H, W, pl, pt, bool(deep_update), md), plans.build_encode_mask, K, h0, w0, H, W, pl, pt,
                     bool(deep_update), md)
        o = eng.pool.get(('emask', K, h, w, eng.devstr),
                         dict(value=((K, h, w, self.value_dim), BF16, False),
                              summ=((K, self.model_cfg['object_summarizer']['num_summaries'], self.embed_dim + 1), F32, False)), dev)
        value, summ = o['value'], o['summ']
        dyn = dict(image=f32c(img), masks=mk, pix_feat=pix, sensory_f32=sf, sensory_bf16=sb, value=value, summ=summ)
        if _split:
            cut = P.meta['value_done']
            P.run_part(0, cut, **dyn)

            def finish():
                P.run_part(cut, None, first=False, **dyn)
                frame_context.remember('sensory_bf16', sf, sb)
                return group_logical(sf), summ.unsqueeze(0)
            return group_logical(value), finish
        P.run(**dyn)
        new_sens = group_logical(sf)
        frame_context.remember('sensory_bf16', sf, sb)
        return group_logical(value), new_sens, summ.unsqueeze(0), None

    def pixel_fusion(self, pix_feat, pixel, sensory, last_mask, *, chunk_size=-1):
        eng = self.engine()
        pf = nhwc_of(pix_feat)
        px = group_nhwc_of(pixel)
        K, h, w = px.shape[:3]
        _, sb = self._sensory_pair(sensory)
        lm = f32c(last_mask[0])
        xt = frame_context.recall('fuse_xt', pf)
        md = frame_context.recall('mask_down', lm)
        md = md is not None and md == (K, h, w, eng.__dict__.get('_md_gen'))
        P = eng.plan(('fuse', K, h, w, xt is not None, md), plans.build_pixel_fusion, K, h, w, xt is not None, md)
        fused = eng.pool.get(('fuse', K, h, w, eng.devstr), dict(fused=((K, h, w, self.embed_dim), BF16, False)), eng.device)['fused']
        P.run(pix_feat=pf, pixel=px, sensory_bf16=sb, last_mask=lm, fused=fused, **({} if xt is None else {'fuse_xt': xt}))
        return group_logical(fused)

    def readout_query(self, pixel_readout, obj_memory, *, selector=None, need_weights=False, _last_aux=True, _summary_token=None):
        assert selector is None, 'selector is a training-time argument'
        eng = self.engine()
        px = group_nhwc_of(pixel_readout)
        K, h, w = px.shape[:3]
        om = obj_memory[0]
        if om.dtype != F32:
            om = om.to(F32)
        om = om.sum(dim=1) if om.shape[1] != 1 else om[:, 0]
        if not om.is_contiguous():
            om = om.contiguous()
        st = eng.__dict__.setdefault('_qinit_state', {})
        fresh = _summary_token is None or st.get(K) != _summary_token or not plans.QINIT_SKIP
        st[K] = _summary_token
        P = eng.plan(('rq', K, h, w, bool(_last_aux), fresh), plans.build_readout_query, K, h, w, bool(_last_aux), fresh)
        out = eng.pool.get(('rq', K, h, w, eng.devstr), dict(out=((K, h, w, self.embed_dim), BF16, False)), eng.device)['out']
        P.run(pixel=px, obj_mem=om, out=out)
        n_aux = P.bufs['aux_logits'].shape[0] - (0 if _last_aux else 1)
        aux = {'logits': [P.bufs['aux_logits'][i].view(1, K, h, w) for i in range(n_aux)],
               'q_weights': None, 'p_weights': None}
        return group_logical(out), aux

    def segment(self, ms_image_feat: List[torch.Tensor], memory_readout, sensory, *, selector=None, chunk_size=-1,
                update_sensory=True, _need_logits=True, _fork=False):
        assert selector is None, 'selector is a training-time argument'
        eng = self.engine()
        dev = eng.device
        p16 = group_nhwc_of(memory_readout)
        K, h, w = p16.shape[:3]
        f8, f4 = nhwc_of(ms_image_feat[1]), nhwc_of(ms_image_feat[2])
        sf, sb = self._sensory_pair(sensory)
        pre = frame_context.recall('decoder_feats', f8)
        if pre is not None and pre[2].data_ptr() != f4.data_ptr():
            pre = None
        md = bool(_fork) and K + 1 <= 8 and dev.type == 'cuda'
        P = eng.plan(('seg', K, h, w, bool(update_sensory), pre is not None, md), plans.build_segment, K, h, w, bool(update_sensory), pre is not None, md)
        sp = dict(prob=((K + 1, 16 * h, 16 * w), F32, False))
        if _need_logits:
            sp['lup'] = ((K + 1, 16 * h, 16 * w), F32, False)
        o = eng.pool.get(('seg', K, h, w, bool(_need_logits), eng.devstr), sp, dev)
        prob, lup = o['prob'], o.get('lup')
        feats = dict(f8=f8, f4=f4) if pre is None else dict(f8p=pre[0], f4p=pre[1])
        dyn = dict(p16=p16, sensory_f32=sf, sensory_bf16=sb, prob=prob, logits_up=lup, **feats)
        n_ops, cut = len(P.ol.recs), P.meta.get('logits_done', 0)
        if _fork and not eng.one_lane and update_sensory and dev.type == 'cuda' and not plans.GRAPHS and 0 < cut < n_ops - 1 and K + 1 <= 16:
            main = torch.cuda.current_stream(dev)
            st = eng.__dict__.setdefault('_streams', {})
            if 'aux' not in st:
                st['aux'] = torch.cuda.Stream(device=dev)
            aux = st['aux']
            P.run_part(0, cut, **dyn)
            aux.wait_stream(main)
            with torch.cuda.stream(aux):
                P.run_part(n_ops - 1, n_ops, first=False)
            P.run_part(cut, n_ops - 1, first=False)
            main.wait_stream(aux)
        else:
            P.run(**dyn)
        new_sens = group_logical(sf)
        frame_context.remember('sensory_bf16', sf, sb)
        if md:
            eng._md_gen = eng.__dict__.get('_md_gen', 0) + 1
            frame_context.remember('mask_down', prob[1:], (K, h, w, eng._md_gen), cap=2)
        else:
            frame_context.forget('mask_down', prob[1:])
        return new_sens, (lup.unsqueeze(0) if lup is not None else None), prob.unsqueeze(0)

    def read_memory(self, *a, **k):
        raise NotImplementedError('read_memory is the training-time path (cutie.py:102-140); inference reads through MemoryManager')

    def compute_aux(self, *a, **k):
        raise NotImplementedError('aux heads are training-only (cutie.py:205-207)')

    def forward(self, *args, **kwargs):
        raise NotImplementedError
```

cutie_amd/model/plans.py:

```python
import math
import os

import numpy as np
import torch

from .. import _lib
from .. import ops as O
from ..ops import Dyn
from .param_spec import resnet_layers

BF16, F32 = torch.bfloat16, torch.float32


class Act:
    __slots__ = ('t', 'B', 'H', 'W', 'C', 'ld')

    def __init__(self, t, B, H, W, C, ld=None):
        self.t, self.B, self.H, self.W, self.C, self.ld = t, B, H, W, C, (C if ld is None else ld)


def positional_encoding(h, w, dim_total, scale, temperature):
    dim = int(math.ceil(dim_total / 4) * 2)
    inv_freq = 1.0 / (temperature ** (torch.arange(0, dim, 2).float() / dim))
    py = torch.arange(h, dtype=torch.float32)
# ... 296 lines not shown
                assert O.korder_class(*best) == want, (key, best, ref)
            if best is None and not getattr(self.eng, 'autotune', AUTOTUNE):
                continue
            if best is None:
                one = arr[n:n + 1].copy()
                best, best_t = (int(i[17]), 1), None
                cands = O.tile_candidates(M, cout, cin, int(i[16]),
                                          geom=dict(kh=int(i[11]), stride=int(i[13]), pad=int(i[14]), W=int(i[2]), c2=int(i[4])))
                if int(i[4]) or arr['p'][n, 4]:
                    cands = [t for t in cands if t != O.COUT1_TILE]
                for t in cands:
                    for sk in O.splitk_candidates(M, cout, int(i[16]), t):
                        one['i'][0, 17], one['i'][0, 19] = t, sk
                        ms = min(ex.time_ops(one, TUNE_ITERS) for _ in range(TUNE_REPS))
                        if best_t is None or ms < best_t:
                            best, best_t = (t, sk), ms
                cache[key] = best
                tuned_any = True
            apply = True
            if (best[0] in O.DMA_TILES or best[0] in O.PC_TILES) and not O.dma_tiles_enabled():
                apply = False
            if (arr['p'][n, 7] or arr['p'][n, 8]) and best[0] not in O.DMA_TILES and best[0] not in O.PC_TILES:
                apply = False
            if apply:
                arr['i'][n, 17], arr['i'][n, 19] = best
            if twin:
                assert O.korder_class(int(arr['i'][n, 17]), int(arr['i'][n, 19])) == want, (key, int(arr['i'][n, 17]), int(arr['i'][n, 19]), want)
        ol.wire_next_weights()
        self.tuned = True
        if tuned_any:
            save_tile_cache(cache)

    def conv(self, wname, x, *, name=None, out=None, stride=1, pad=None, x2=None, res=None, res_bcast=False,
             relu_in=False, act=O.ACT_NONE, out_f32=False, ldy=None, gap_acc=None, zero=None, persistent=False, res_group=None):
        w = self.eng.w[wname]
        if pad is None:
            pad = (w.kh - 1) // 2
        OH = (x.H + 2 * pad - w.kh) // stride + 1
        OW = (x.W + 2 * pad - w.kw) // stride + 1
        if out is None:
            t = self.buf(name or wname, (x.B, OH, OW, w.cout), F32 if out_f32 else BF16, persistent=persistent)
            out = Act(t, x.B, OH, OW, w.cout, w.cout if ldy is None else ldy)
        else:
            assert out.B == x.B and out.H == OH and out.W == OW and out.C == w.cout, (wname, out.B, out.H, out.W, out.C, OH, OW, w.cout)
        if res is not None:
            assert res.C == w.cout and res.H == OH and res.W == OW

        def emit(s0, s1, zero):
            whole = s0 == 0 and s1 == x.B
            cut = (lambda a, elem: a.t) if whole else (lambda a, elem: _objects_from(a, s0, elem))
            return self.ol.conv(cut(x, 2), w, cut(out, 4 if out_f32 else 2), B=s1 - s0, H=x.H, W=x.W, C1=x.C, ldx1=x.ld, OH=OH, OW=OW, ldy=out.ld, stride=stride,
                                pad=pad, x2=None if x2 is None else cut(x2, 2), C2=0 if x2 is None else x2.C,
                                ldx2=0 if x2 is None else x2.ld, res=None if res is None else (res.t if res_bcast else cut(res, 2)),
                                ldr=0 if res is None else res.ld, res_bcast=res_bcast, relu_in=relu_in, act=act, out_f32=out_f32,
                                gap_acc=gap_acc if (gap_acc is None or whole) else gap_acc[s0:], zero=zero, prio=self.prio, res_group=res_group)
        if self.mixed is None or x.B != sum(self.mixed):
            emit(0, x.B, zero)
            return out
        assert res_group is None
        counts, st = self.mixed, O.clip_starts(self.mixed)
        side = gap_acc is not None or zero is not None
        cin = x.C + (0 if x2 is None else x2.C)

        def one_clip_class(Kc):
            M1 = Kc * OH * OW
            key1 = O.conv_tile_key(M1, w.cout, cin, w.kh, stride, relu_in, out_f32, x.H, x.W)
            static = O.static_tile(M1, w.cout, cin, w.kh, 0 if x2 is None else x2.C, res is not None, side)
            return O.korder_class(*(self.eng.tile_cache.get(key1) or (static, 1)))
        cls = [one_clip_class(k) for k in counts]
        c0 = 0
        for c in range(1, len(counts) + 1):
            if c < len(counts) and cls[c] == cls[c0]:
                continue
            z = zero
            if zero is not None and c - c0 < len(counts):
                per_obj = zero.dim() == 2 and zero.shape[0] == x.B
                z = zero[st[c0]:st[c]] if per_obj else (zero if c0 == 0 else None)
            n = emit(st[c0], st[c], z)
            if c - c0 > 1:
                self.kref[n] = counts[c0]
            c0 = c
        return out

    def ca_block(self, prefix, x, name, out=None, head=None):
        if head is not None:
            head = (self.eng.w[head[0]], head[1])
        w = self.eng.w[prefix + '.conv2']
        gap = self.buf(name + '.gap', (x.B, x.C), F32)
        HW = x.H * x.W
        if O.conv_side_jobs_ok(cin=x.C, cout=w.cout, kh=w.kh):
            sums = self.buf(name + '.gapsum', (x.B, x.C), torch.int64)
            t1 = self.conv(prefix + '.conv1', x, name=name + '.t1', relu_in=True, act=O.ACT_RELU, zero=sums)
            t2 = self.conv(prefix + '.conv2', t1, name=name + '.t2', gap_acc=sums)
            if out is None:
                out = Act(self.buf(name + '.out', (x.B, x.H, x.W, x.C)), x.B, x.H, x.W, x.C)
            self.ol.eca_apply(t2.t, gap, self.eng.w[prefix + '.conv.weight'], x.t, out.t, B=x.B, HW=HW, C=x.C, fixed_sums=sums, head=head)
            return out
        t1 = self.conv(prefix + '.conv1', x, name=name + '.t1', relu_in=True, act=O.ACT_RELU)
        t2 = self.conv(prefix + '.conv2', t1, name=name + '.t2')
        self.ol.gap(t2.t, gap, B=x.B, HW=HW, C=x.C, partial_only=True)
        if out is None:
            out = Act(self.buf(name + '.out', (x.B, x.H, x.W, x.C)), x.B, x.H, x.W, x.C)
        self.ol.eca_apply(t2.t, gap, self.eng.w[prefix + '.conv.weight'], x.t, out.t, B=x.B, HW=HW, C=x.C, head=head)
        return out

    def fusion_block(self, prefix, x, g, name, out=None, xt=None, xt_group=None):
        if xt is None:
            xt = self.conv(prefix + '.distributor.x_transform', x, name=name + '.xt')
        if xt_group is not None and not isinstance(xt_group[0], int):
            counts, stride = xt_group
            xte = self.buf(name + '.xte', (g.B, xt.H, xt.W, xt.C))
            self.ol.copy2d(xt.t, xte, rows=g.B, rowbytes=xt.H * xt.W * xt.C * 2, src_stride=stride * xt.ld * 2, dst_stride=xt.H * xt.W * xt.C * 2, clips=counts)
            g0 = self.conv(prefix + '.distributor.g_transform', g, name=name + '.g0', res=Act(xte, g.B, xt.H, xt.W, xt.C))
        else:
            g0 = self.conv(prefix + '.distributor.g_transform', g, name=name + '.g0', res=xt, res_bcast=True, res_group=xt_group)
        g1 = self.ca_block(prefix + '.block1', g0, name + '.b1')
        return self.ca_block(prefix + '.block2', g1, name + '.b2', out=out)

    def resnet(self, prefix, x, taps=None):
        bottleneck, layers = resnet_layers(self.eng.m, prefix)
        feats = {}
        for (lname, planes, nb, lstride) in layers:
            for bi in range(nb):
                p = f'{prefix}.{lname}.{bi}'
                s = lstride if bi == 0 else 1
                last = bi == nb - 1
                out = taps.get(lname) if (taps and last) else None
                if bottleneck:
                    t1 = self.conv(p + '.conv1', x, act=O.ACT_RELU)
                    t2 = self.conv(p + '.conv2', t1, stride=s, act=O.ACT_RELU)
                    r = self.conv(p + '.downsample.0', x, stride=s) if (p + '.downsample.0') in self.eng.w else x
                    x = self.conv(p + '.conv3', t2, res=r, act=O.ACT_RELU, out=out)
                else:
                    t1 = self.conv(p + '.conv1', x, stride=s, act=O.ACT_RELU)
                    r = self.conv(p + '.downsample.0', x, stride=s) if (p + '.downsample.0') in self.eng.w else x
                    x = self.conv(p + '.conv2', t1, res=r, act=O.ACT_RELU, out=out)
            feats[lname] = x
        return x, feats


def _objects_from(a, s0, elem):
    per_obj = a.H * a.W * a.ld
    if isinstance(a.t, Dyn):
        return Dyn(a.t.name, a.t.offset + s0 * per_obj * elem)
    assert a.t.is_contiguous() and a.t.element_size() == elem, (a.t.shape, a.t.dtype, elem)
    return a.t.reshape(-1)[s0 * per_obj:]


MIXED_FUSION_EXTRA = 1


def clip_layout(K, clips):
    if isinstance(clips, int):
        counts = (int(K),) * clips
    else:
        counts = tuple(int(k) for k in clips)
    return len(counts), counts, O.clip_starts(counts), len(set(counts)) > 1


def stem_ok(eng, name):
    w = eng.w.get(name)
    return w is not None and w.cout == 64 and w.kh == 7 and w.kw == 7 and w.cin_padded == 8 and w.bias is not None


def build_encode(eng, h0, w0, H, W, pad_left, pad_top, B=1, qrows=64):
    P = Plan(eng, touch=weights_go_cold(B * (H // 16) * (W // 16)), prio=False)
    m = eng.m
    img = (lambda b: Dyn('image')) if B == 1 else (lambda b: Dyn('image%d' % b))
    if stem_ok(eng, 'pixel_encoder.conv1'):
        pool = P.buf('pool', (B, H // 4, W // 4, 64))
        SM = O.OpList.STEM_MAX_IMAGES
        for b0 in range(0, B, SM):
            P.ol.stem(img(b0), None, eng.w['pixel_encoder.conv1'], pool[b0:], h0=h0, w0=w0, H=H, W=W, pad_left=pad_left, pad_top=pad_top, K=1,
                      mean=m['pixel_mean'], std=m['pixel_std'], relu=True, more_images=[img(b) for b in range(b0 + 1, min(B, b0 + SM))])
        x = Act(pool, B, H // 4, W // 4, 64)
    else:
        img8 = P.buf('img8', (B, H, W, 8))
        for b in range(B):
            P.ol.img_prep(img(b), None, img8[b], h0=h0, w0=w0, H=H, W=W, pad_left=pad_left, pad_top=pad_top, K=1,
                          mean=m['pixel_mean'], std=m['pixel_std'])
        x = P.conv('pixel_encoder.conv1', Act(img8, B, H, W, 8), stride=2, pad=3, act=O.ACT_RELU)
        pool = P.buf('pool', (B, x.H // 2, x.W // 2, 64))
        P.ol.maxpool(x.t, pool, B=B, H=x.H, W=x.W, C=64)
        x = Act(pool, B, x.H // 2, x.W // 2, 64)
    h4, w4, h8, w8, h, w = H // 4, W // 4, H // 8, W // 8, H // 16, W // 16
    ms = m['pixel_encoder']['ms_dims']
    taps = {'res2': Act(Dyn('f4'), B, h4, w4, ms[2]), 'layer2': Act(Dyn('f8'), B, h8, w8, ms[1]),
            'layer3': Act(Dyn('f16'), B, h, w, ms[0])}
    f16, _ = P.resnet('pixel_encoder', x, taps)
    pix = P.conv('pix_feat_proj', f16, out=Act(Dyn('pix_feat'), B, h, w, m['pixel_dim']))
    build_key_ops(P, f16, h, w, qrows)
    W_ = eng.w
    for wname, src, dname in (('mask_decoder.decoder_feat_proc.transforms.0', taps['layer2'], 'f8p'),
                              ('mask_decoder.decoder_feat_proc.transforms.1', taps['res2'], 'f4p'),
                              ('pixel_fuser.fuser.distributor.x_transform', pix, 'fuse_xt')):
        P.conv(wname, src, out=Act(Dyn(dname), B, src.H, src.W, W_[wname].cout))
    P.meta.update(h=h, w=w, B=B)
    if B > 1:
        P.korder_ref = B
    return P


def build_key_ops(P, f16, h, w, qrows=64):
    m = P.eng.m
    CK = m['key_dim']
    B = f16.B
    kx = P.conv('key_proj.pix_feat_proj', f16, name='keyx')
    P.conv('key_proj.key_proj', kx, out=Act(Dyn('key'), B, h, w, CK), out_f32=True)
    P.conv('key_proj.d_proj', kx, out=Act(Dyn('shr'), B, h, w, 1), out_f32=True, act=O.ACT_SQ1)
    P.conv('key_proj.e_proj', kx, out=Act(Dyn('sel'), B, h, w, CK), out_f32=True, act=O.ACT_SIGMOID)
    hw, HWp = h * w, -(-h * w // qrows) * qrows
    for b in range(B):
        P.ol.key_prep(Dyn('key', b * hw * CK * 4), Dyn('sel', b * hw * CK * 4), Dyn('Bhi', b * HWp * 128 * 2), Dyn('Blo', b * HWp * 128 * 2),
                      Dyn('cq', b * HWp * 4), n=hw, query=True)


def build_transform_key(eng, h, w):
    P = Plan(eng)
    build_key_ops(P, Act(Dyn('f16'), 1, h, w, eng.m['pixel_encoder']['ms_dims'][0]), h, w)
    return P


def build_pixel_fusion(eng, K, h, w, pre=False, pre_md=False, clips=1, wstride=1, stacked=False):
    G, counts, st, mixed = clip_layout(K, clips)
    gkey = counts if mixed else G
    K = st[-1]
    assert G == 1 or pre, 'clips in lock step take x_transform(pix_feat) from the encoder plan'
    assert not (mixed and stacked), 'the joint read-out pass writes uniform groups only'
    P = Plan(eng, touch=weights_go_cold(h * w, K))
    P.mixed = counts if mixed else None
    m = eng.m
    if pre_md:
        pair = eng.mask_down_bufs(K, h, w, gkey)[0]
        P.ol.keep.append(pair)
    else:
        pair = P.buf('pair', (K, h, w, 64), persistent=True)
        m16 = P.buf('m16', (K, h, w), F32)
        for c in range(G):
            P.ol.mask_down(Dyn('last_mask' if G == 1 else 'last_mask%d' % c), pair[st[c]:], m16[st[c]:], K=counts[c], H=16 * h, W=16 * w, pair_channels=64)
    if G > 1 and not stacked:
        px = P.buf('pixel_all', (K, h, w, m['value_dim']))
        nb = h * w * m['value_dim'] * 2
        P.ol.bank_write([(Dyn('pixel%d' % c), px[st[c]:], counts[c] * nb) for c in range(G)])
        pixel = Act(px, K, h, w, m['value_dim'])
    else:
        pixel = Act(Dyn('pixel'), K, h, w, m['value_dim'])
    p16 = P.conv('pixel_fuser.sensory_compress', Act(Dyn('sensory_bf16'), K, h, w, m['sensory_dim']),
                 x2=Act(pair, K, h, w, 64), res=pixel, name='p16')
    xt = Act(Dyn('fuse_xt'), G, h, w, eng.w['pixel_fuser.fuser.distributor.x_transform'].cout) if pre else None
    P.fusion_block('pixel_fuser.fuser', Act(Dyn('pix_feat'), 1, h, w, m['pixel_dim']), p16, 'fuse',
                   out=Act(Dyn('fused'), K, h, w, m['embed_dim']), xt=xt, xt_group=(counts if mixed else counts[0], wstride * h * w) if G > 1 else None)
    if G > 1 and not mixed:
        P.korder_ref = G
    return P


def build_readout_query(eng, K, h, w, last_aux=True, fresh=True, clips=1):
    G, counts, st, mixed = clip_layout(K, clips)
    K = st[-1]
    Kc = counts if mixed else counts[0]
    P = Plan(eng, touch=weights_go_cold(h * w, K))
    P.mixed = counts if mixed else None
    if G > 1 and not mixed:
        P.korder_ref = G
    m, ol, W = eng.m, P.ol, eng.w
    ot = m['object_transformer']
    C, Q, heads, nb = m['embed_dim'], ot['num_queries'], ot['num_heads'], ot['num_blocks']
    HW, M = h * w, K * Q
    t = 'object_transformer'
    f = lambda name, shape: P.buf(name, shape, F32)
    query, query_emb = eng.query_bufs(K)
    use_chain = C == 256 and Q == 16 and heads == 8 and HW <= 24576 and ot['ff_dim'] % 64 == 0
    assert G == 1 or use_chain, 'clips in lock step need the chain form of the query side'
    qacc = P.buf('qacc', (3 * nb, M, C), torch.int64) if use_chain else None
    zero_on_conv = None
    if C == 256 and Q == 16:
        if fresh or not use_chain:
            ol.query_init2(Dyn('obj_mem'), query, query_emb, rows=M, w_init=W[t + '.summary_to_query_init'], res_init=eng.rep_embedding('query_init', K),
                           w_emb=W[t + '.summary_to_query_emb'], res_emb=eng.rep_embedding('query_emb', K), zero=qacc)
        elif O.conv_side_jobs_ok(cin=C, cout=C, kh=1):
            zero_on_conv = qacc
        else:
            ol.memset32(qacc, 2 * qacc.numel(), 0)
    else:
        vals = f('vals', (M, C))
        ol.query_init(Dyn('obj_mem'), vals, rows=M, C=C)
        ol.linear(vals, W[t + '.summary_to_query_init'], query, M=M, res=eng.rep_embedding('query_init', K))
        ol.linear(vals, W[t + '.summary_to_query_emb'], query_emb, M=M, res=eng.rep_embedding('query_emb', K))
    pix_in = Act(Dyn('pixel'), K, h, w, C)
    pixel = P.conv(t + '.pixel_init_proj', pix_in, name='pixel_init', zero=zero_on_conv)
    aux = P.buf('aux_logits', (nb + 1, K, HW), F32, persistent=True)
    fused_mask = HW <= 24576
    fg = None if fused_mask else P.buf('fg', (K, HW), torch.uint8)
    nfg = None if fused_mask else P.buf('nfg', (K,), torch.int32)
    P.conv(t + '.mask_pred.0.1', pixel, relu_in=True, out_f32=True, out=Act(aux[0], K, h, w, 1))
    if not fused_mask:
        ol.aux_mask(aux[0], fg, nfg, K=K, HW=HW)
    x = query
    prev_acc = q_pre = xn_next = None
    for b in range(nb):
        q = f'{t}.blocks.{b}'
        n = f'b{b}.'
        kvq = P.conv(q + '.pixel_proj_x', pixel, x2=pix_in, name=n + 'kvq', res=Act(eng.pe_rb(h, w, b), 1, h, w, 3 * C), res_bcast=True)
        ln = lambda name: (W[q + name + '.weight'], W[q + name + '.bias'])
        xn = xn_next if xn_next is not None else f(n + 'xn', (M, C))
        xn_next = None
        fuse_proj = fused_mask and C == 256
        chain = fuse_proj and use_chain
        if chain:
            Wo1, Wo2 = W[q + '.read_from_pixel.out'], W[q + '.self_attn.out']
            W1, W2 = W[q + '.ffn.linear1'], W[q + '.ffn.linear2']
            a1, a2, a3 = qacc[3 * b], qacc[3 * b + 1], qacc[3 * b + 2]
            if q_pre is not None:
                ol.attn_q2p(None, kvq.t, None, None, None, K=K, Q=Q, HW=HW, C=C, heads=heads, ldkv=3 * C, voff=C, logits=aux[b],
                            q_pre=q_pre, out_proj=(Wo1, a1), clip_objects=Kc)
            else:
                ol.attn_q2p(None, kvq.t, None, None, None, K=K, Q=Q, HW=HW, C=C, heads=heads, ldkv=3 * C, voff=C, logits=aux[b],
                            proj=dict(x=x, W=W[q + '.read_from_pixel.q'], emb=query_emb, ln=ln('.read_from_pixel.norm'), ln_out=xn),
                            acc_in=prev_acc, out_proj=(Wo1, a1), clip_objects=Kc)
            y = f(n + 'y', (M, C))
            ol.attn_self(None, None, None, K=K, Q=Q, C=C, heads=heads,
                         proj=dict(x=xn, W=W[q + '.self_attn.qkv'], emb=query_emb, ln=ln('.self_attn.norm'), ln_out=y),
                         acc_in=(a1, Wo1.bias), out_proj=(Wo2, a2))
            x2 = f(n + 'x2', (M, C))
            ol.qffn(y, x2, a3, rows=M, ln=ln('.ffn.norm'), W1=W1, W2=W2, acc_in=(a2, Wo2.bias), hid_slice=64)
            x = x2
            prev_acc = (a3, W2.bias)
            next_q = None
            if b + 1 < nb:
                qn = f'{t}.blocks.{b + 1}'
                q_pre, xn_next = f(f'b{b + 1}.q', (M, C)), f(f'b{b + 1}.xn', (M, C))
                next_q = dict(ln=(W[qn + '.read_from_pixel.norm.weight'], W[qn + '.read_from_pixel.norm.bias']), W=W[qn + '.read_from_pixel.q'],
                              q_out=q_pre, xn_out=xn_next)
            else:
                q_pre = None
            pa = P.buf(n + 'pa', (K, h, w, C))
            ol.attn_p2q(kvq.t.view(-1)[2 * C:], None, None, pa, K=K, Q=Q, HW=HW, C=C, heads=heads, ldq=3 * C,
                        proj=dict(x=x, W=W[q + '.read_from_query.kv'], emb=query_emb), acc_in=prev_acc, next_q=next_q)
        else:
            att = f(n + 'att', (M, C))
            if fuse_proj:
                ol.attn_q2p(None, kvq.t, None, None, att, K=K, Q=Q, HW=HW, C=C, heads=heads, ldkv=3 * C, voff=C, logits=aux[b],
                            proj=dict(x=x, W=W[q + '.read_from_pixel.q'], emb=query_emb, ln=ln('.read_from_pixel.norm'), ln_out=xn))
            else:
                qp = f(n + 'qp', (M, C))
                ol.linear(x, W[q + '.read_from_pixel.q'], qp, M=M, x_add=query_emb, add_rows=M, ln=ln('.read_from_pixel.norm'), ln_out=xn)
                ol.attn_q2p(qp, kvq.t, fg, nfg, att, K=K, Q=Q, HW=HW, C=C, heads=heads, ldkv=3 * C, voff=C, logits=aux[b] if fused_mask else None)
            x1 = f(n + 'x1', (M, C))
            ol.linear(att, W[q + '.read_from_pixel.out'], x1, M=M, res=xn)
            y = f(n + 'y', (M, C))
            sa = f(n + 'sa', (M, C))
            if fuse_proj:
                ol.attn_self(None, None, sa, K=K, Q=Q, C=C, heads=heads,
                             proj=dict(x=x1, W=W[q + '.self_attn.qkv'], emb=query_emb, ln=ln('.self_attn.norm'), ln_out=y))
            else:
                qkv = f(n + 'qkv', (M, 3 * C))
                ol.linear(x1, W[q + '.self_attn.qkv'], qkv, M=M, x_add=query_emb, add_rows=M, add_cols=2 * C, ln=ln('.self_attn.norm'), ln_out=y)
                ol.attn_self(qkv, qkv.view(-1)[2 * C:], sa, K=K, Q=Q, C=C, heads=heads, ldqk=3 * C, ldv=3 * C)
            x2 = f(n + 'x2', (M, C))
            ol.linear(sa, W[q + '.self_attn.out'], x2, M=M, res=y)
            hid = f(n + 'hid', (M, ot['ff_dim']))
            ol.linear(x2, W[q + '.ffn.linear1'], hid, M=M, relu=True, ln=ln('.ffn.norm'))
            x3 = f(n + 'x3', (M, C))
            ol.linear(hid, W[q + '.ffn.linear2'], x3, M=M, res=x2)
            x = x3
            pa = P.buf(n + 'pa', (K, h, w, C))
            if fuse_proj:
                ol.attn_p2q(kvq.t.view(-1)[2 * C:], None, None, pa, K=K, Q=Q, HW=HW, C=C, heads=heads, ldq=3 * C,
                            proj=dict(x=x, W=W[q + '.read_from_query.kv'], emb=query_emb))
            else:
                kv2 = f(n + 'kv2', (M, 2 * C))
                ol.linear(x, W[q + '.read_from_query.kv'], kv2, M=M, x_add=query_emb, add_rows=M, add_cols=C)
                ol.attn_p2q(kvq.t.view(-1)[2 * C:], kv2, kv2.view(-1)[C:], pa, K=K, Q=Q, HW=HW, C=C, heads=heads, ldq=3 * C, ldkv=2 * C)
        pf = P.conv(q + '.read_from_query.out', Act(pa, K, h, w, C), name=n + 'pf', res=pixel)
        last = b == nb - 1
        want_aux = not last or last_aux
        fuse_head = want_aux and C == 256
        pixel = P.ca_block(q + '.pixel_ffn.conv', pf, n + 'ffn', out=Act(Dyn('out'), K, h, w, C) if last else None,
                           head=(f'{t}.mask_pred.{b + 1}.1', aux[b + 1]) if fuse_head else None)
        if want_aux and not fuse_head:
            P.conv(f'{t}.mask_pred.{b + 1}.1', pixel, relu_in=True, out_f32=True, out=Act(aux[b + 1], K, h, w, 1))
        if not last and not fused_mask:
            ol.aux_mask(aux[b + 1], fg, nfg, K=K, HW=HW)
    return P


def build_segment(eng, K, h, w, update_sensory, pre=False, md=False, clips=1, wstride=1):
    G, counts, st, mixed = clip_layout(K, clips)
    K = st[-1]
    Kc = max(counts)
    assert G == 1 or (pre and Kc + 1 <= 8), 'clips in lock step: image-only decoder convs from the encoder plan, <= 7 objects per clip'
    P = Plan(eng, touch=weights_go_cold(h * w, K))
    P.mixed = counts if mixed else None
    gkey = counts if mixed else G
    sgrp = counts if mixed else counts[0]
    if G > 1 and not mixed:
        P.korder_ref = G
    m, ol = eng.m, P.ol
    up = m['mask_decoder']['up_dims']
    ms = m['pixel_encoder']['ms_dims']
    CS = m['sensory_dim']
    h8, w8, h4, w4 = 2 * h, 2 * w, 4 * h, 4 * w
    if pre:
        f8p, f4p = Act(Dyn('f8p'), G, h8, w8, up[0]), Act(Dyn('f4p'), G, h4, w4, up[1])
    else:
        f8p = P.conv('mask_decoder.decoder_feat_proc.transforms.0', Act(Dyn('f8'), 1, h8, w8, ms[1]), name='f8p')
        f4p = P.conv('mask_decoder.decoder_feat_proc.transforms.1', Act(Dyn('f4'), 1, h4, w4, ms[2]), name='f4p')
    p16 = Act(Dyn('p16'), K, h, w, up[0])
    u8 = P.buf('u8', (K, h8, w8, up[0]))
    ol.upsample2x_add(p16.t, f8p.t, u8, B=K, h=h, w=w, C=up[0], skip_group=(sgrp, wstride * h8 * w8) if G > 1 else None)
    u8 = Act(u8, K, h8, w8, up[0])
    t1 = P.conv('mask_decoder.up_16_8.out_conv.conv1', u8, relu_in=True, act=O.ACT_RELU)
    ds = P.conv('mask_decoder.up_16_8.out_conv.downsample', u8)
    p8 = P.conv('mask_decoder.up_16_8.out_conv.conv2', t1, res=ds, name='p8')
    u4 = P.buf('u4', (K, h4, w4, up[1]))
    ol.upsample2x_add(p8.t, f4p.t, u4, B=K, h=h8, w=w8, C=up[1], skip_group=(sgrp, wstride * h4 * w4) if G > 1 else None)
    u4 = Act(u4, K, h4, w4, up[1])
    t2 = P.conv('mask_decoder.up_8_4.out_conv.conv1', u4, relu_in=True, act=O.ACT_RELU)
    p4 = P.conv('mask_decoder.up_8_4.out_conv.conv2', t2, res=u4, name='p4')
    logits = P.buf('logits', (K, h4, w4), F32)
    P.conv('mask_decoder.pred', p4, relu_in=True, out_f32=True, out=Act(logits, K, h4, w4, 1))
    P.meta['logits_done'] = len(ol.recs)
    if update_sensory:
        CT = up[1] + up[2] + 64
        gcat = P.buf('gcat', (K, h, w, CT), persistent=True)
        ol.area_down3([dict(x=p8.t, y=gcat, B=K, H=h8, W=w8, C=up[1], ldx=up[1], ldy=CT, r=2),
                       dict(x=p4.t, y=gcat.view(-1)[up[1]:], B=K, H=h4, W=w4, C=up[2], ldx=up[2], ldy=CT, r=4),
                       dict(x=logits, y=gcat.view(-1)[up[1] + up[2]:], B=K, H=h4, W=w4, C=1, ldx=1, ldy=CT, r=4, f32_in=True, Cz=8)])
        g3 = P.conv('mask_decoder.sensory_update.g_all', p16, x2=Act(gcat, K, h, w, CT), name='g3')
        vals = P.conv('mask_decoder.sensory_update.transform', g3, x2=Act(Dyn('sensory_bf16'), K, h, w, CS),
                      out_f32=True, name='gru_vals')
        ol.gru(vals.t, Dyn('sensory_f32'), Dyn('sensory_bf16'), n=K * h * w, C=CS)
    if Kc + 1 <= 16:
        ol.up4_softmax(logits, Dyn('prob'), Dyn('logits_up'), P=Kc + 1, h=h4, w=w4, from_logits=True, clips=counts if mixed else G,
                       mask_down=(eng.mask_down_bufs(K, h, w, gkey)[1], eng.mask_down_bufs(K, h, w, gkey)[0], 64) if md else None)
    else:
        agg = P.buf('agg', (K + 1, h4, w4), F32)
        ol.seg_agg(logits, agg, K=K, hw=h4 * w4)
        ol.up4_softmax(agg, Dyn('prob'), Dyn('logits_up'), P=K + 1, h=h4, w=w4)
    return P


def build_encode_mask(eng, K, h0, w0, H, W, pad_left, pad_top, deep_update=True, pre_md=False, clips=1, wstride=1):
    G, counts, st, mixed = clip_layout(K, clips)
    K = st[-1]
    Kc = counts[0]
    P = Plan(eng, touch=weights_go_cold((H // 16) * (W // 16), K))
    P.mixed = counts if mixed else None
    if G > 1 and not mixed:
        P.korder_ref = G
    m, ol = eng.m, P.ol
    h, w = H // 16, W // 16
    CV, CS, CE, Q = m['value_dim'], m['sensory_dim'], m['embed_dim'], m['object_summarizer']['num_summaries']
    masks_of = (lambda c: Dyn('masks')) if G == 1 else (lambda c: Dyn('masks', 4 * (st[c] + c + 1) * H * W))
    assert G == 1 or stem_ok(eng, 'mask_encoder.conv1')
    if stem_ok(eng, 'mask_encoder.conv1'):
        pool = P.buf('pool', (K, H // 4, W // 4, 64))
        iname = lambda c: Dyn('image' if G == 1 else 'image%d' % c)
        SM = O.OpList.STEM_MAX_IMAGES
        for c0 in range(0, G, SM):
            ol.stem(iname(c0), masks_of(c0), eng.w['mask_encoder.conv1'], pool[st[c0]:], h0=h0, w0=w0, H=H, W=W, pad_left=pad_left, pad_top=pad_top,
                    K=Kc, mean=m['pixel_mean'], std=m['pixel_std'], relu=True, more_images=[iname(c) for c in range(c0 + 1, min(G, c0 + SM))],
                    mask_stride=(Kc + 1) * H * W, counts=counts if mixed else None)
    else:
        x8 = P.buf('x8', (K, H, W, 8))
        ol.img_prep(Dyn('image'), Dyn('masks'), x8, h0=h0, w0=w0, H=H, W=W, pad_left=pad_left, pad_top=pad_top, K=K,
                    mean=m['pixel_mean'], std=m['pixel_std'])
        x = P.conv('mask_encoder.conv1', Act(x8, K, H, W, 8), stride=2, pad=3)
        pool = P.buf('pool', (K, x.H // 2, x.W // 2, 64))
        ol.maxpool(x.t, pool, B=K, H=x.H, W=x.W, C=64, relu=True)
    g16, _ = P.resnet('mask_encoder', Act(pool, K, H // 4, W // 4, 64))
    xt = xt_group = None
    if G > 1:
        wx = eng.w['mask_encoder.fuser.distributor.x_transform']
        xt_t = P.buf('fuse.xt', (G, h, w, wx.cout))
        for c in range(G):
            P.conv('mask_encoder.fuser.distributor.x_transform', Act(Dyn('pix_feat', 2 * c * wstride * h * w * m['pixel_dim']), 1, h, w, m['pixel_dim']),
                   out=Act(xt_t[c:c + 1], 1, h, w, wx.cout))
        xt, xt_group = Act(xt_t, G, h, w, wx.cout), (counts if mixed else Kc, h * w)
    value = P.fusion_block('mask_encoder.fuser', Act(Dyn('pix_feat'), 1, h, w, m['pixel_dim']), g16, 'fuse',
                           out=Act(Dyn('value'), K, h, w, CV), xt=xt, xt_group=xt_group)
    P.meta['value_done'] = len(ol.recs)
    if deep_update:
        vals = P.conv('mask_encoder.sensory_update.transform', value, x2=Act(Dyn('sensory_bf16'), K, h, w, CS),
                      out_f32=True, name='gru_vals')
        ol.gru(vals.t, Dyn('sensory_f32'), Dyn('sensory_bf16'), n=K * h * w, C=CS)
    if pre_md:
        m16 = eng.mask_down_bufs(K, h, w, counts if mixed else G)[1]
    else:
        pair = P.buf('pair', (K, h, w, 8))
        m16 = P.buf('m16', (K, h, w), F32)
        for c in range(G):
            ol.mask_down(masks_of(c), pair[st[c]:], m16[st[c]:], K=counts[c], H=H, W=W)
# ... 14 lines not shown
```

cutie_amd/ops.py:

```python
import os

import numpy as np
import torch

from . import _lib

NI, NF, NP = 24, 6, 16
OP_DTYPE = np.dtype([('kind', '<i4'), ('flags', '<i4'), ('i', '<i4', (NI,)), ('f', '<f4', (NF,)), ('p', '<u8', (NP,))])
assert OP_DTYPE.itemsize == _lib.OP_STRUCT_SIZE

(CONV, MAXPOOL, IMG_PREP, UPSAMPLE2X_ADD, AREA_DOWN, MASK_DOWN, GAP, ECA_APPLY, GRU, SEG_AGG, UP4_SOFTMAX,
 MASK_MERGE, AGG_SOFTMAX, LINEAR, LAYERNORM, QUERY_INIT, AUX_MASK, ATTN_Q2P, ATTN_SELF, ATTN_P2Q, SUMMARIZE,
 ADD_PE, KEY_PREP, AFF_SCORE, AFF_SELECT, AFF_READOUT, MEMSET32, COPY2D, AXPY, USAGE_TICK, RANK_SELECT,
 GATHER_ROWS, CONSOL_AFF, CONSOL_READ, CAST, PROB_TO_ID, RESIZE, FLIP_W, AREA_DOWN3, QFFN, STEM, BANK_WRITE) = range(1, 43)

KIND_NAMES = {}
for _n in ('CONV MAXPOOL IMG_PREP UPSAMPLE2X_ADD AREA_DOWN MASK_DOWN GAP ECA_APPLY GRU SEG_AGG UP4_SOFTMAX MASK_MERGE '
           'AGG_SOFTMAX LINEAR LAYERNORM QUERY_INIT AUX_MASK ATTN_Q2P ATTN_SELF ATTN_P2Q SUMMARIZE ADD_PE KEY_PREP '
           'AFF_SCORE AFF_SELECT AFF_READOUT MEMSET32 COPY2D AXPY USAGE_TICK RANK_SELECT GATHER_ROWS CONSOL_AFF '
           'CONSOL_READ CAST PROB_TO_ID RESIZE FLIP_W AREA_DOWN3 QFFN STEM').split():
    KIND_NAMES[globals()[_n]] = _n

F_RELU_IN, F_OUT_F32, F_RES_BCAST = 1, 2, 4
F_PRIO, F_AFF_PRIO = 256, 64
F_TILE_OFF = 128 if os.environ.get('CUTIE_AMD_COUT1_TILE', '1') in ('', '0') else 0
ACT_NONE, ACT_RELU, ACT_SIGMOID, ACT_SQ1 = 0, 1, 2, 3
ACT_SHIFT = 4
AREA_RT = 8 if os.environ.get('CUTIE_AMD_AREA_R', '1') in ('', '0') else 0
GRU_SCALAR = 1 if os.environ.get('CUTIE_AMD_GRU4', '1') in ('', '0') else 0
KEYPREP_LOOP = 2 if os.environ.get('CUTIE_AMD_KEYPREP_LOOP', '0') not in ('', '0') else 0
UP4_LANES = 16 if os.environ.get('CUTIE_AMD_UP4_SHARED', '1') in ('', '0') else 0
SELECT_COARSE = 2 if os.environ.get('CUTIE_AMD_SELECT_FINE', '1') in ('', '0') else 0
UP4_RTK = 8 if os.environ.get('CUTIE_AMD_UP4_KC', '1') in ('', '0') else 0

TILES = {0: (128, 128, 32), 1: (128, 64, 32), 2: (64, 64, 32), 3: (256, 16, 32), 4: (64, 128, 32),
         5: (64, 64, 64), 6: (64, 128, 64), 7: (128, 128, 64), 8: (64, 64, 128), 9: (32, 64, 64),
         10: (128, 64, 64), 11: (32, 64, 128), 12: (32, 128, 64),
         13: (64, 64, 64), 14: (128, 64, 64), 15: (64, 128, 64), 16: (128, 128, 64), 17: (64, 64, 128), 18: (128, 128, 32),
         20: (64, 64, 64), 21: (64, 64, 128), 22: (32, 64, 128), 23: (128, 64, 64), 24: (64, 128, 64), 25: (128, 128, 64),
         26: (32, 64, 64), 27: (64, 64, 64), 28: (32, 64, 64), 29: (64, 128, 32), 30: (64, 64, 32)}
TILE_WK = {20: 2, 21: 2, 22: 2, 23: 2, 24: 2, 25: 2, 26: 2, 27: 4, 28: 4, 29: 2, 30: 2}

DMA_TILES = {60: (128, 128, 64), 61: (128, 128, 64), 62: (128, 128, 64), 63: (128, 64, 64), 64: (64, 128, 64), 65: (64, 64, 64),
             66: (64, 64, 64), 67: (32, 64, 64), 68: (256, 128, 64), 69: (32, 128, 64), 70: (128, 128, 64), 71: (128, 64, 64),
             72: (64, 64, 64), 73: (64, 64, 64), 74: (64, 64, 64), 75: (32, 64, 64), 76: (128, 64, 64), 77: (64, 128, 64), 78: (32, 128, 64),
             80: (64, 64, 128), 81: (64, 64, 128), 82: (32, 64, 128), 83: (32, 64, 128), 84: (64, 128, 128), 85: (128, 64, 128),
             86: (96, 64, 64), 87: (96, 64, 64), 88: (64, 64, 64), 89: (64, 64, 64)}


PC_TILES = {100: (64, 64, 64), 101: (64, 64, 64), 102: (32, 64, 64), 103: (128, 64, 64), 104: (64, 128, 64), 105: (128, 128, 64),
            106: (128, 128, 64), 107: (64, 64, 64), 108: (128, 128, 64), 109: (32, 64, 64), 110: (96, 64, 64), 111: (96, 128, 64),
            120: (64, 64, 64), 121: (64, 64, 64), 122: (128, 64, 64), 123: (128, 128, 64), 124: (64, 128, 64), 125: (32, 64, 64),
            126: (128, 128, 64), 127: (64, 128, 64), 129: (96, 64, 64), 130: (32, 64, 64), 131: (64, 128, 64),
            132: (64, 64, 64), 133: (96, 128, 64), 134: (320, 64, 64),
            140: (64, 64, 64), 141: (96, 64, 64), 142: (96, 64, 64), 143: (32, 64, 64), 144: (128, 64, 64),
            145: (96, 64, 64), 146: (128, 64, 64), 147: (32, 64, 64)}
PC_HALO = {120: (8, 8), 121: (4, 16), 122: (8, 16), 123: (8, 16), 124: (8, 8), 125: (4, 8), 126: (8, 16), 127: (4, 16),
           129: (10, 9), 130: (5, 6), 131: (6, 9), 132: (6, 9), 133: (10, 9), 134: (20, 16),
           145: (10, 9), 146: (8, 16), 147: (5, 6)}

ALL_TILES = {**TILES, **DMA_TILES, **PC_TILES}


def korder_class(tile, splitk=1):
    if tile in PC_HALO:
        return 'halo'
    if tile in TILE_WK or splitk != 1:
        return ('split', tile, splitk)
    if tile in (3, COUT1_TILE):
        return ('small', tile)
    return 'stream' if (tile in DMA_TILES or tile in PC_TILES) else 'igemm'


def pc_tile_ok(tile, *, cin, kh, stride=1, pad=None, c2=0):
    if cin % 64 or (c2 and (c2 % 64 or (cin - c2) % 64)) or kh > 5:
        return False
    if tile in PC_HALO:
        return kh == 3 and stride == 1 and (pad is None or pad == 1)
    return True


def pc_blocks(tile, B, OH, OW, cout):
    bm, bn, _ = PC_TILES[tile]
    if tile in PC_HALO:
        th, tw = PC_HALO[tile]
        return B * -(-OH // th) * -(-OW // tw) * -(-cout // bn)
    return -(-(B * OH * OW) // bm) * -(-cout // bn)


def dma_tiles_enabled():
    return os.environ.get('CUTIE_AMD_DMA_TILES', '1') not in ('', '0')


def dma_tile_ok(tile, *, cin, kh, c2=0):
    bk = DMA_TILES[tile][2]
    return cin % bk == 0 and (c2 == 0 or (c2 % bk == 0 and (cin - c2) % bk == 0)) and kh * kh <= 32


def conv_side_jobs_ok(*, cin, cout, kh, c2=0):
    return dma_tiles_enabled() and dma_tile_ok(60, cin=cin, kh=kh, c2=c2) and cout % 8 == 0 and cout > 16


NUM_CU = 256
WEIGHT_PREFETCH = int(os.environ.get('CUTIE_AMD_WPF', str(8 << 20)))
WEIGHT_PREFETCH_BLOCK = int(os.environ.get('CUTIE_AMD_WPF_BLOCK', str(48 << 10)))


COUT1_TILE = 19


# ... 243 lines not shown
            self.finalize()
        words = self._words
        if words is None:
            assert OP_DTYPE.itemsize == 256 and OP_DTYPE.fields['p'][1] == 128
            words = self._words = ({name: tuple((idx * 32 + 16 + slot, off) for (idx, slot, off) in sl) for name, sl in self.dyn.items()},
                                   memoryview(self.arr).cast('B').cast('Q'))
        table, mv = words
        for name, t in tensors.items():
            sl = table.get(name)
            if sl is None:
                continue
            base = 0 if t is None else (t if type(t) is int else t.data_ptr())
            if base:
                for w, off in sl:
                    mv[w] = base + off
            else:
                for w, off in sl:
                    mv[w] = 0

    def run(self, _stream=None, **tensors):
        if self.arr is None:
            self.finalize()
        if tensors:
            self.bind(**tensors)
        ex = _lib.get_executor()
        if _stream is None:
            ex.run(self.arr)
        elif hasattr(ex, 'run_on'):
            ex.run_on(self.arr, _stream)
        else:
            with torch.cuda.stream(_stream):
                ex.run(self.arr)

    def __len__(self):
        return len(self.recs)

    def conv(self, x1, w, y, *, B, H, W, C1, ldx1, OH, OW, ldy, stride=1, pad=0, x2=None, C2=0, ldx2=0,
             res=None, ldr=0, res_bcast=False, relu_in=False, act=ACT_NONE, out_f32=False, tile=None, splitk=1,
             gap_acc=None, zero=None, prio=False, res_group=None):
        flags = (F_RELU_IN if relu_in else 0) | (F_OUT_F32 if out_f32 else 0) | (F_RES_BCAST if res_bcast else 0) | (act << ACT_SHIFT) | F_TILE_OFF | \
            (F_PRIO if prio else 0)
        assert C1 + C2 == w.cin_padded, (C1, C2, w.cin_padded)
        M = B * OH * OW
        side = gap_acc is not None or zero is not None
        if tile is None:
            tile = static_tile(M, w.cout, C1 + C2, w.kh, C2, res is not None, side)
        if side:
            assert (tile in DMA_TILES or tile in PC_TILES) and not out_f32 and w.cout % 8 == 0 and ldy % 8 == 0, 'GAP accumulation needs an LDS-DMA conv (see conv_side_jobs_ok)'
        part = splitk_scratch(w.weight.device, self.scratch_owner)
        self.wbytes[len(self.recs)] = w.weight.numel() * w.weight.element_size()
        return self.add(CONV, flags,
                        [B, H, W, C1, C2, ldx1, ldx2, OH, OW, w.cout, ldy, w.kh, w.kw, stride, pad, ldr, w.kpad, tile, w.cin_real,
                         splitk, part.numel() // 1024, 0 if zero is None else zero.numel()],
                        self._res_group(res_group, res_bcast, B, OH * OW), [x1, x2, w.weight, w.bias, res, y, part, gap_acc, zero])

    @staticmethod
    def _res_group(res_group, res_bcast, B, OHW):
        if res_group is None:
            return []
        kg, stride = int(res_group[0]), int(res_group[1])
        assert res_bcast and kg > 0 and B % kg == 0 and stride >= OHW and stride < (1 << 24), (res_group, B, OHW)
        return [float(kg), float(stride)]

    def maxpool(self, x, y, *, B, H, W, C, relu=False):
        OH, OW = (H + 2 - 3) // 2 + 1, (W + 2 - 3) // 2 + 1
        return self.add(MAXPOOL, 1 if relu else 0, [B, H, W, C, OH, OW], [], [x, y])

    STEM_MAX_IMAGES = 12

    def stem(self, image, masks, w, y, *, h0, w0, H, W, pad_left, pad_top, K, mean, std, relu=True, more_images=(), mask_stride=0, counts=None):
        assert w.cout == 64 and w.kh == 7 and w.cin_padded == 8 and H % 16 == 0 and W % 16 == 0
        more = list(more_images)
        assert len(more) < self.STEM_MAX_IMAGES
        if counts is not None:
            assert len(counts) == 1 + len(more) and len(counts) > 1
            ints = [h0, w0, H, W, pad_left, pad_top, max(counts), w.kpad, len(counts), 0, pack_counts(counts)]
            return self.add(STEM, 1 if relu else 0, ints, list(mean) + list(std), [image, masks, w.weight, w.bias, y] + more)
        ints = [h0, w0, H, W, pad_left, pad_top, K, w.kpad] + ([1 + len(more), int(mask_stride)] if more else [])
        return self.add(STEM, 1 if relu else 0, ints, list(mean) + list(std), [image, masks, w.weight, w.bias, y] + more)

    def img_prep(self, image, masks, y, *, h0, w0, H, W, pad_left, pad_top, K, mean, std):
        return self.add(IMG_PREP, 0, [h0, w0, H, W, pad_left, pad_top, K], list(mean) + list(std), [image, masks, y])

    def upsample2x_add(self, g, skip, y, *, B, h, w, C, skip_group=None):
        ints = [B, h, w, C]
        if skip_group is not None and not isinstance(skip_group[0], int):
            counts, stride = skip_group
            assert sum(counts) == B and stride >= 4 * h * w
            ints += [0, int(stride), pack_counts(counts)]
        elif skip_group is not None:
            kg, stride = int(skip_group[0]), int(skip_group[1])
            assert kg > 0 and B % kg == 0 and stride >= 4 * h * w
            ints += [kg, stride]
        return self.add(UPSAMPLE2X_ADD, 0, ints, [], [g, skip, y])

    def area_down(self, x, y, *, B, H, W, C, ldx, ldy, r, f32_in=False, Cz=None):
        return self.add(AREA_DOWN, 1 if f32_in else 0, [B, H, W, C, ldx, ldy, r, C if Cz is None else Cz], [], [x, y])

    def area_down3(self, segs):
        assert len(segs) == 3
        ints, ptrs, flags = [], [], 0
        for q, g in enumerate(segs):
            ints += [g['B'], g['H'], g['W'], g['C'], g['ldx'], g['ldy'], g['r'], g['C'] if g.get('Cz') is None else g['Cz']]
            ptrs += [g['x'], g['y']]
            flags |= (1 << q) if g.get('f32_in') else 0
        return self.add(AREA_DOWN3, flags | AREA_RT, ints, [], ptrs)

    def mask_down(self, masks, pair, m16, *, K, H, W, r=16, pair_channels=8):
        assert pair_channels % 8 == 0
        return self.add(MASK_DOWN, 0, [K, H, W, r, pair_channels], [], [masks, pair, m16])

    def gap(self, x, y, *, B, HW, C, scratch=None, partial_only=False):
        if scratch is None:
            scratch = torch.zeros((B, -(-HW // 64), C), dtype=torch.float32, device=y.device)
        self._last_gap_scratch = scratch
        return self.add(GAP, 1 if partial_only else 0, [B, HW, C], [], [x, y, scratch])

    def eca_apply(self, x, gap, wk, r, y, *, B, HW, C, part=None, fixed_sums=None, head=None):
        tail = []
        if head is not None:
            w, out = head
            assert C == 256 and w.cout == 1 and w.kh == 1 and w.cin_padded == 256
            tail = [w.weight, w.bias, out]
        if fixed_sums is not None:
            return self.add(ECA_APPLY, 1, [B, HW, C], [], [x, gap, wk, r, y, fixed_sums] + tail)
        if part is None:
            part = self._last_gap_scratch
        return self.add(ECA_APPLY, 0, [B, HW, C], [], [x, gap, wk, r, y, part] + tail)

    def gru(self, values, h, hb, *, n, C):
        return self.add(GRU, GRU_SCALAR, [n, C], [], [values, h, hb])

    def seg_agg(self, logits, agg, *, K, hw):
        return self.add(SEG_AGG, 0, [K, hw], [], [logits, agg])

    def up4_softmax(self, agg, prob, logits_up, *, P, h, w, from_logits=False, mask_down=None, clips=1):
        if not isinstance(clips, int):
            counts = [int(k) for k in clips]
            assert from_logits and len(counts) > 1 and h % 4 == 0 and w % 4 == 0 and not UP4_RTK, 'the mixed form: compile-time object counts'
            ints = [max(counts) + 1, h, w, 0, len(counts), pack_counts(counts)]
            if mask_down is not None:
                m16, pair, ints[3] = mask_down
                return self.add(UP4_SOFTMAX, 1 | 4 | UP4_LANES, ints, [], [agg, prob, logits_up, m16, pair])
            return self.add(UP4_SOFTMAX, 1, ints, [], [agg, prob, logits_up])
        if mask_down is not None:
            assert from_logits and P <= 8 and h % 4 == 0 and w % 4 == 0
            m16, pair, pitch = mask_down
            return self.add(UP4_SOFTMAX, 1 | 4 | UP4_RTK | UP4_LANES, [P, h, w, pitch, clips], [], [agg, prob, logits_up, m16, pair])
        assert clips == 1 or (from_logits and P <= 8)
        return self.add(UP4_SOFTMAX, (1 | UP4_RTK) if from_logits else 0, [P, h, w, 0, clips], [], [agg, prob, logits_up])

    def mask_merge(self, inmask, pred, src, planes, *, h0, w0, H, W, pad_left, pad_top, Knew, Kold, nfloat, float_mode):
        return self.add(MASK_MERGE, 1 if float_mode else 0, [h0, w0, H, W, pad_left, pad_top, Knew, Kold, nfloat], [],
                        [inmask, pred, src, planes])

    def agg_softmax(self, planes, prob, *, K, HW):
        return self.add(AGG_SOFTMAX, 0, [K, HW], [], [planes, prob])

    def linear(self, x, w, y, *, M, ldx=None, ldy=None, x_add=None, add_rows=0, res=None, relu=False, add_cols=0,
               ln=None, ln_out=None, eps=1e-5):
        flags = (1 if relu else 0) | (2 if ln is not None else 0)
        return self.add(LINEAR, flags,
                        [M, w.n, w.kd, w.kd if ldx is None else ldx, w.n if ldy is None else ldy, add_rows, add_cols], [eps],
                        [x, x_add, w.weight, w.bias, res, y, ln[0] if ln else None, ln[1] if ln else None, ln_out])

    def layernorm(self, x, g, b, y, *, M, C):
        return self.add(LAYERNORM, 0, [M, C], [], [x, g, b, y])

    def query_init(self, obj_mem, y, *, rows, C):
        return self.add(QUERY_INIT, 0, [rows, C], [], [obj_mem, y])

    def query_init2(self, obj_mem, query, query_emb, *, rows, w_init, res_init, w_emb, res_emb, zero=None):
        assert w_init.kd == 256 and w_init.n == 256 and w_emb.kd == 256 and w_emb.n == 256 and rows % 16 == 0
        nz = 0
        if zero is not None:
            nb = zero.numel() * zero.element_size()
            assert nb % 16 == 0 and zero.is_contiguous()
# ... 596 lines not shown
```

Baseline: 1173.

## Fold final ECA channel-attention apply into segment decoder's upsample2x_add kernel

Result: slower. 1160 (-1.1%).

```diff
diff --git a/cutie_amd/_lib.py b/cutie_amd/_lib.py
--- a/cutie_amd/_lib.py
+++ b/cutie_amd/_lib.py
@@ -69,6 +69,10 @@
 
 def has_track_stats():
     return bool(load().cutie_hip_build_flags() & 16)
+
+
+def has_eca_fold():
+    return bool(load().cutie_hip_build_flags() & 32)
 
 
 class HipExecutor:
diff --git a/cutie_amd/csrc/api.hip b/cutie_amd/csrc/api.hip
--- a/cutie_amd/csrc/api.hip
+++ b/cutie_amd/csrc/api.hip
@@ -127,7 +127,7 @@
 int cutie_hip_abi_version(void) { return 11; }
 int cutie_op_struct_size(void) { return (int)sizeof(cutie_op); }
 int cutie_hip_build_flags(void) {
-    const int forms = 2 | 4 | 8 | 16;
+    const int forms = 2 | 4 | 8 | 16 | 32;
 #ifdef CUTIE_DIAG
     return forms | 1;
 #else
diff --git a/cutie_amd/csrc/eca.h b/cutie_amd/csrc/eca.h
--- /dev/null
+++ b/cutie_amd/csrc/eca.h
@@ -0,0 +1,44 @@
+#pragma once
+#include "common.h"
+
+__device__ __forceinline__ float eca_mean_fixed(long long sum, float inv_hw) {
+    return (float)((double)sum * (1.0 / 16777216.0)) * inv_hw;
+}
+
+__device__ __forceinline__ float eca_scale(const float* __restrict__ wk, const float* gap, int c) {
+    const float a = wk[0] * gap[c] + wk[1] * gap[c + 1] + wk[2] * gap[c + 2] + wk[3] * gap[c + 3] + wk[4] * gap[c + 4];
+    return sigmoidf_(a);
+}
+
+__device__ __forceinline__ int eca_sc_slot(int c) { return (c & 7) * 32 + (c >> 3); }
+
+__device__ __forceinline__ uint32_t eca_apply_pair(uint32_t x, uint32_t r, const float* sc, int i, int c8) {
+    const float lo = __uint_as_float(x << 16) * sc[(2 * i) * 32 + c8] + __uint_as_float(r << 16);
+    const float hi = __uint_as_float(x & 0xffff0000u) * sc[(2 * i + 1) * 32 + c8] + __uint_as_float(r & 0xffff0000u);
+    return pack_bf2(lo, hi);
+}
+
+__device__ __forceinline__ uint4 eca_apply_octet(const uint4& x, const uint4& r, const float* sc, int c8) {
+    const uint32_t* xu = &x.x; const uint32_t* ru = &r.x;
+    return make_uint4(eca_apply_pair(xu[0], ru[0], sc, 0, c8), eca_apply_pair(xu[1], ru[1], sc, 1, c8),
+                      eca_apply_pair(xu[2], ru[2], sc, 2, c8), eca_apply_pair(xu[3], ru[3], sc, 3, c8));
+}
+
+__device__ __forceinline__ float eca_head_part(const uint32_t* st, const uint32_t* wu) {
+    float part = 0.f;
+#pragma unroll
+    for (int i = 0; i < 4; ++i) {
+        part += fmaxf(__uint_as_float(st[i] << 16), 0.f) * __uint_as_float(wu[i] << 16);
+        part += fmaxf(__uint_as_float(st[i] & 0xffff0000u), 0.f) * __uint_as_float(wu[i] & 0xffff0000u);
+    }
+    return part;
+}
+__device__ __forceinline__ float eca_head_sum32(float part) {
+    part += __uint_as_float(__builtin_amdgcn_update_dpp(0, (int)__float_as_uint(part), 0xB1, 0xf, 0xf, false));
+    part += __uint_as_float(__builtin_amdgcn_update_dpp(0, (int)__float_as_uint(part), 0x4E, 0xf, 0xf, false));
+    part += __uint_as_float(__builtin_amdgcn_update_dpp(0, (int)__float_as_uint(part), 0x141, 0xf, 0xf, false));
+    part += __uint_as_float(__builtin_amdgcn_update_dpp(0, (int)__float_as_uint(part), 0x140, 0xf, 0xf, false));
+    const unsigned pu = __float_as_uint(part);
+    const auto rr = __builtin_amdgcn_permlane16_swap(pu, pu, false, false);
+    return __uint_as_float(rr[0]) + __uint_as_float(rr[1]);
+}
diff --git a/cutie_amd/csrc/elementwise.hip b/cutie_amd/csrc/elementwise.hip
--- a/cutie_amd/csrc/elementwise.hip
+++ b/cutie_amd/csrc/elementwise.hip
@@ -1,4 +1,5 @@
 #include "common.h"
+#include "eca.h"
 #include <math.h>
 
 #define GRID1D(n, bs) dim3((unsigned)(((long)(n) + (bs) - 1) / (bs)))
@@ -64,6 +65,23 @@
     if (i0 > n_in - 1) i0 = n_in - 1;
     i1 = i0 + (i0 < n_in - 1 ? 1 : 0);
     lam = src - (float)i0;
+}
+
+__device__ __forceinline__ uint4 up2_blend(const uint4& v00, const uint4& v01, const uint4& v10, const uint4& v11, const uint4& sk, float ly, float lx) {
+    const uint32_t* a = &v00.x; const uint32_t* bq = &v01.x; const uint32_t* cq = &v10.x; const uint32_t* d = &v11.x;
+    const uint32_t* s = &sk.x;
+    float w00 = (1.f - ly) * (1.f - lx), w01 = (1.f - ly) * lx, w10 = ly * (1.f - lx), w11 = ly * lx;
+    uint32_t out[4];
+#pragma unroll
+    for (int i = 0; i < 4; ++i) {
+        float lo = w00 * __uint_as_float(a[i] << 16) + w01 * __uint_as_float(bq[i] << 16) +
+                   w10 * __uint_as_float(cq[i] << 16) + w11 * __uint_as_float(d[i] << 16) + __uint_as_float(s[i] << 16);
+        float hi = w00 * __uint_as_float(a[i] & 0xffff0000u) + w01 * __uint_as_float(bq[i] & 0xffff0000u) +
+                   w10 * __uint_as_float(cq[i] & 0xffff0000u) + w11 * __uint_as_float(d[i] & 0xffff0000u) +
+                   __uint_as_float(s[i] & 0xffff0000u);
+        out[i] = pack_bf2(lo, hi);
+    }
+    return make_uint4(out[0], out[1], out[2], out[3]);
 }
 
 template <bool MIXED = false>
@@ -86,20 +104,61 @@
     if (MIXED) { int st; grp = mixed_clip_of((unsigned)Kg, b, st); }
     else grp = Kg > 0 ? b / Kg : 0;
     uint4 sk = skip[(grp * gstride + (long)oy * OW + ox) * C8 + c];
-    const uint32_t* a = &v00.x; const uint32_t* bq = &v01.x; const uint32_t* cq = &v10.x; const uint32_t* d = &v11.x;
-    const uint32_t* s = &sk.x;
-    float w00 = (1.f - ly) * (1.f - lx), w01 = (1.f - ly) * lx, w10 = ly * (1.f - lx), w11 = ly * lx;
-    uint32_t out[4];
-#pragma unroll
-    for (int i = 0; i < 4; ++i) {
-        float lo = w00 * __uint_as_float(a[i] << 16) + w01 * __uint_as_float(bq[i] << 16) +
-                   w10 * __uint_as_float(cq[i] << 16) + w11 * __uint_as_float(d[i] << 16) + __uint_as_float(s[i] << 16);
-        float hi = w00 * __uint_as_float(a[i] & 0xffff0000u) + w01 * __uint_as_float(bq[i] & 0xffff0000u) +
-                   w10 * __uint_as_float(cq[i] & 0xffff0000u) + w11 * __uint_as_float(d[i] & 0xffff0000u) +
-                   __uint_as_float(s[i] & 0xffff0000u);
-        out[i] = pack_bf2(lo, hi);
-    }
-    y[idx] = make_uint4(out[0], out[1], out[2], out[3]);
+    y[idx] = up2_blend(v00, v01, v10, v11, sk, ly, lx);
+}
+
+template <bool MIXED = false>
+__global__ __launch_bounds__(256) void upsample2x_add_eca_kernel(const uint4* __restrict__ t2, const uint4* __restrict__ r,
+                                                                 const long long* __restrict__ fixed, const float* __restrict__ wk,
+                                                                 uint4* __restrict__ g, const uint4* __restrict__ skip, uint4* __restrict__ y,
+                                                                 float* __restrict__ gap_out, const bf16_t* __restrict__ pw,
+                                                                 const float* __restrict__ pb, float* __restrict__ plog,
+                                                                 int B, int h, int w, int Kg, long gstride, int prio) {
+    if (prio) __builtin_amdgcn_s_setprio(1);
+    constexpr int C8 = 32, C = 256;
+    __shared__ float gap[2][C + 4], sc[2][C];
+    const int tid = threadIdx.x;
+    const int OH = 2 * h, OW = 2 * w;
+    const long per = (long)OH * OW * C8, total = (long)B * per;
+    const long idx0 = (long)blockIdx.x * 256;
+    const bool valid = idx0 + tid < total;
+    const long idx = valid ? idx0 + tid : total - 1;
+    const int b0 = (int)(idx0 / per), b1 = (int)(min(idx0 + 255, total - 1) / per);
+    const int c = idx % C8; long t = idx / C8;
+    const int ox = t % OW; t /= OW; const int oy = t % OH; const int b = t / OH;
+    int y0, y1, x0, x1; float ly, lx;
+    up_coord(oy, h, 0.5f, y0, y1, ly);
+    up_coord(ox, w, 0.5f, x0, x1, lx);
+    const long ob = (long)b * h * w * C8;
+    const long o00 = ob + ((long)y0 * w + x0) * C8 + c, o01 = ob + ((long)y0 * w + x1) * C8 + c;
+    const long o10 = ob + ((long)y1 * w + x0) * C8 + c, o11 = ob + ((long)y1 * w + x1) * C8 + c;
+    const uint4 a00 = t2[o00], a01 = t2[o01], a10 = t2[o10], a11 = t2[o11];
+    const uint4 r00 = r[o00], r01 = r[o01], r10 = r[o10], r11 = r[o11];
+    long grp;
+    if (MIXED) { int st; grp = mixed_clip_of((unsigned)Kg, b, st); }
+    else grp = Kg > 0 ? b / Kg : 0;
+    const uint4 sk = skip[(grp * gstride + (long)oy * OW + ox) * C8 + c];
+    const float inv = 1.f / (float)(h * w);
+    for (int q = 0; q <= b1 - b0; ++q) {
+        const float mean = eca_mean_fixed(fixed[(long)(b0 + q) * C + tid], inv);
+        gap[q][tid + 2] = mean;
+        if (gap_out && (q == 1 || idx0 == b0 * per)) gap_out[(long)(b0 + q) * C + tid] = mean;
+    }
+    if (tid < 2) { gap[0][tid] = gap[1][tid] = 0.f; gap[0][C + 2 + tid] = gap[1][C + 2 + tid] = 0.f; }
+    __syncthreads();
+    for (int q = 0; q <= b1 - b0; ++q) sc[q][eca_sc_slot(tid)] = eca_scale(wk, gap[q], tid);
+    __syncthreads();
+    const float* s = sc[b - b0];
+    const uint4 v00 = eca_apply_octet(a00, r00, s, c), v01 = eca_apply_octet(a01, r01, s, c);
+    const uint4 v10 = eca_apply_octet(a10, r10, s, c), v11 = eca_apply_octet(a11, r11, s, c);
+    const bool own = valid && (oy & 1) && (ox & 1);
+    if (valid) y[idx] = up2_blend(v00, v01, v10, v11, sk, ly, lx);
+    if (own) g[o00] = v00;
+    if (pw) {
+        const uint4 wv = *reinterpret_cast<const uint4*>(pw + c * 8);
+        const float tot = eca_head_sum32(eca_head_part(&v00.x, &wv.x));
+        if (own && c == 0) plog[(long)b * h * w + (long)y0 * w + x0] = tot + (pb ? pb[0] : 0.f);
+    }
 }
 
 template <int R = 0>
@@ -323,7 +382,7 @@
     }
     if (fixed) {
         for (int c = tid; c < C; c += 256) {
-            const float mean = (float)((double)fixed[(long)b * C + c] * (1.0 / 16777216.0)) * inv;
+            const float mean = eca_mean_fixed(fixed[(long)b * C + c], inv);
             gap[c + 2] = mean;
             if (gap_out && blockIdx.x == 0) gap_out[(long)b * C + c] = mean;
         }
@@ -342,10 +401,7 @@
     }
     if (tid < 2) { gap[tid] = 0.f; gap[C + 2 + tid] = 0.f; }
     __syncthreads();
-    for (int c = tid; c < C; c += 256) {
-        float a = wk[0] * gap[c] + wk[1] * gap[c + 1] + wk[2] * gap[c + 2] + wk[3] * gap[c + 3] + wk[4] * gap[c + 4];
-        sc[(c & 7) * 32 + (c >> 3)] = sigmoidf_(a);
-    }
+    for (int c = tid; c < C; c += 256) sc[eca_sc_slot(c)] = eca_scale(wk, gap, c);
     __syncthreads();
 #pragma unroll
     for (int it = 0; it < 4; ++it) {
@@ -355,11 +411,7 @@
         const uint32_t* xu = &xv[it].x; const uint32_t* ru = &rv[it].x;
         uint32_t o[4];
 #pragma unroll
-        for (int i = 0; i < 4; ++i) {
-            float lo = __uint_as_float(xu[i] << 16) * sc[(2 * i) * 32 + c8] + __uint_as_float(ru[i] << 16);
-            float hi = __uint_as_float(xu[i] & 0xffff0000u) * sc[(2 * i + 1) * 32 + c8] + __uint_as_float(ru[i] & 0xffff0000u);
-            o[i] = pack_bf2(lo, hi);
-        }
+        for (int i = 0; i < 4; ++i) o[i] = eca_apply_pair(xu[i], ru[i], sc, i, c8);
         *reinterpret_cast<uint4*>(y + offs[it]) = make_uint4(o[0], o[1], o[2], o[3]);
     }
     if (pw) {
@@ -372,22 +424,12 @@
             float part = 0.f;
             if (offs[it] >= 0) {
                 const uint32_t* xu = &xv[it].x; const uint32_t* ru = &rv[it].x;
-#pragma unroll
-                for (int i = 0; i < 4; ++i) {
-                    const float lo = __uint_as_float(xu[i] << 16) * sc[(2 * i) * 32 + c8] + __uint_as_float(ru[i] << 16);
-                    const float hi = __uint_as_float(xu[i] & 0xffff0000u) * sc[(2 * i + 1) * 32 + c8] + __uint_as_float(ru[i] & 0xffff0000u);
-                    const uint32_t st = pack_bf2(lo, hi);
-                    part += fmaxf(__uint_as_float(st << 16), 0.f) * __uint_as_float(wu[i] << 16);
-                    part += fmaxf(__uint_as_float(st & 0xffff0000u), 0.f) * __uint_as_float(wu[i] & 0xffff0000u);
-                }
-            }
-            part += __uint_as_float(__builtin_amdgcn_update_dpp(0, (int)__float_as_uint(part), 0xB1, 0xf, 0xf, false));
-            part += __uint_as_float(__builtin_amdgcn_update_dpp(0, (int)__float_as_uint(part), 0x4E, 0xf, 0xf, false));
-            part += __uint_as_float(__builtin_amdgcn_update_dpp(0, (int)__float_as_uint(part), 0x141, 0xf, 0xf, false));
-            part += __uint_as_float(__builtin_amdgcn_update_dpp(0, (int)__float_as_uint(part), 0x140, 0xf, 0xf, false));
-            const unsigned pu = __float_as_uint(part);
-            const auto rr = __builtin_amdgcn_permlane16_swap(pu, pu, false, false);
-            const float tot = __uint_as_float(rr[0]) + __uint_as_float(rr[1]);
+                uint32_t st[4];
+#pragma unroll
+                for (int i = 0; i < 4; ++i) st[i] = eca_apply_pair(xu[i], ru[i], sc, i, c8);
+                part = eca_head_part(st, wu);
+            }
+            const float tot = eca_head_sum32(part);
             const int q = tid + it * 256, p = p0 + q / C8;
             if (c8 == 0 && offs[it] >= 0) plog[(long)b * HW + p] = tot + bias;
         }
@@ -1361,6 +1403,20 @@
         case CUTIE_OP_UPSAMPLE2X_ADD: {
             int C8 = i[3] / 8;
             long n = (long)i[0] * 4 * i[1] * i[2] * C8;
+            if (op->flags & 1) {
+                if (i[3] != 256 || (long)i[1] * i[2] < 2 || !p[3] || !p[4] || !p[5] || !p[6] || (p[8] && !p[10])) {
+                    cutie_set_error("upsample2x_add (ECA form): C = 256, h * w >= 2, t2 / r / sums / conv1d weights (and an output for the head)"); return -2; }
+                int objs = i[0];
+                const bool mixed = i[6] != 0;
+                if (mixed ? (mixed_clips((unsigned)i[6], &objs) < 1 || objs != i[0] || i[4] != 0 || i[5] < 4 * i[1] * i[2])
+                          : (i[4] < 0 || (i[4] > 0 && (i[0] % i[4] || i[5] < 4 * i[1] * i[2])))) {
+                    cutie_set_error("upsample2x_add (ECA form): the skip groups do not fit B = %d (or their stride is below one map)", i[0]); return -2; }
+                auto kern = mixed ? upsample2x_add_eca_kernel<true> : upsample2x_add_eca_kernel<false>;
+                hipLaunchKernelGGL(kern, GRID1D(n, 256), dim3(256), 0, s, (const uint4*)p[3], (const uint4*)p[4], (const long long*)p[5], (const float*)p[6],
+                                   (uint4*)p[0], (const uint4*)p[1], (uint4*)p[2], (float*)p[7], (const bf16_t*)p[8], (const float*)p[9], (float*)p[10],
+                                   i[0], i[1], i[2], mixed ? i[6] : i[4], (long)i[5], PRIO);
+                break;
+            }
             if (i[6]) {
                 int objs; const int nc = mixed_clips((unsigned)i[6], &objs);
                 if (nc < 1 || objs != i[0] || i[4] != 0 || i[5] < 4 * i[1] * i[2]) { cutie_set_error("upsample2x_add (mixed form): the counts 0x%x do not add up to B = %d (or i4 != 0, or the stride is below one map)", i[6], i[0]); return -2; }
diff --git a/cutie_amd/inference/inference_core.py b/cutie_amd/inference/inference_core.py
--- a/cutie_amd/inference/inference_core.py
+++ b/cutie_amd/inference/inference_core.py
@@ -402,8 +402,10 @@
             log.warning('Trying to segment without any memory!')
             return torch.zeros((1, key.shape[-2] * 16, key.shape[-1] * 16), device=key.device, dtype=key.dtype)
         ids = self.object_manager.all_obj_ids
-        memory_readout = self.memory.read(pix_feat, key, selection, self.last_mask, self.network)
+        memory_readout = self.memory.read(pix_feat, key, selection, self.last_mask, self.network, defer_out=True)
         stacked = self.memory.readout_stacked(ids)
+        if stacked is None:
+            self.network.finish_readout()
         memory_readout = stacked if stacked is not None else self.object_manager.realize_dict(memory_readout)
         sensory, _, pred_prob_with_bg = self.network.segment(ms_features, memory_readout, self.memory.get_sensory(ids),
                                                              chunk_size=self.chunk_size, update_sensory=update_sensory,
diff --git a/cutie_amd/inference/lockstep.py b/cutie_amd/inference/lockstep.py
--- a/cutie_amd/inference/lockstep.py
+++ b/cutie_amd/inference/lockstep.py
@@ -371,12 +371,14 @@
         token = tuple(core.memory._objv_token for core in cores)
         fresh = token != self._qtoken or not plans.QINIT_SKIP
         self._qtoken = token
-        P = eng.plan(('ls_rq',) + lay + (h, w, fresh), plans.build_readout_query, K, h, w, False, fresh, clips)
+        fold = plans.eca_fold_ok(eng, m['embed_dim'], h * w)
+        P = eng.plan(('ls_rq',) + lay + (h, w, fresh, fold), plans.build_readout_query, K, h, w, False, fresh, clips, fold)
         out = eng.pool.get(('ls_rq',) + lay + (h, w, eng.devstr), dict(out=((KT, h, w, m['embed_dim']), BF16, False)), dev)['out']
         P.run(pixel=fused, obj_mem=ov, out=out)
-        P = eng.plan(('ls_seg',) + lay + (h, w, bool(update_sensory), ws), plans.build_segment, K, h, w, bool(update_sensory), True, True, clips, ws)
+        eca = {'eca_' + k: P.bufs[P.meta['eca'][k]] for k in ('t2', 'r', 'sums')} if fold else {}
+        P = eng.plan(('ls_seg',) + lay + (h, w, bool(update_sensory), ws, fold), plans.build_segment, K, h, w, bool(update_sensory), True, True, clips, ws, fold)
         prob = eng.pool.get(('ls_seg',) + lay + (h, w, eng.devstr), dict(prob=((KT + G, 16 * h, 16 * w) if mixed else (G, K + 1, 16 * h, 16 * w), F32, False)), dev)['prob']
-        P.run(p16=out, sensory_f32=sf, sensory_bf16=sb, prob=prob, logits_up=None, f8p=recs[0]['f8p'], f4p=recs[0]['f4p'])
+        P.run(p16=out, sensory_f32=sf, sensory_bf16=sb, prob=prob, logits_up=None, f8p=recs[0]['f8p'], f4p=recs[0]['f4p'], **eca)
         self._md_valid = True
         probs = [prob[st[c] + c:st[c + 1] + c + 1] for c in range(G)] if mixed else [prob[c] for c in range(G)]
         for c, core in enumerate(cores):
diff --git a/cutie_amd/inference/memory_manager.py b/cutie_amd/inference/memory_manager.py
--- a/cutie_amd/inference/memory_manager.py
+++ b/cutie_amd/inference/memory_manager.py
@@ -453,7 +453,7 @@
         return out
 
     def read(self, pix_feat: torch.Tensor, query_key: torch.Tensor, selection: torch.Tensor, last_mask: torch.Tensor,
-             network) -> Dict[int, torch.Tensor]:
+             network, defer_out: bool = False) -> Dict[int, torch.Tensor]:
         q = network.query_operands(query_key, selection)
         h, w = pix_feat.shape[-2:]
         dev = pix_feat.device
@@ -473,7 +473,8 @@
                 a, b = self._rows(objects, self._objv_ids)
                 this_obj_mem = self._objv[a:b].unsqueeze(0).unsqueeze(2)
                 readout_memory, aux_features = network.readout_query(pixel_readout, this_obj_mem, _last_aux=self.save_aux,
-                                                                     _summary_token=(self._objv_token, a, b))
+                                                                     _summary_token=(self._objv_token, a, b),
+                                                                     _defer_out=defer_out and len(self.buckets) == 1 and cs >= K)
                 for i, obj in enumerate(objects):
                     all_readout[obj] = readout_memory[:, i]
                 chunks.append((objects, readout_memory))
diff --git a/cutie_amd/model/cutie.py b/cutie_amd/model/cutie.py
--- a/cutie_amd/model/cutie.py
+++ b/cutie_amd/model/cutie.py
@@ -196,6 +196,7 @@
         e.__dict__.pop('_query_bufs', None)
         e.__dict__.pop('_md_bufs', None)
         e.__dict__.pop('_qinit_state', None)
+        e.__dict__.pop('_eca_pending', None)
         return e
 
     def plan(self, key, builder, *args):
@@ -520,11 +521,13 @@
         P.run(pix_feat=pf, pixel=px, sensory_bf16=sb, last_mask=lm, fused=fused, **({} if xt is None else {'fuse_xt': xt}))
         return group_logical(fused)
 
-    def readout_query(self, pixel_readout, obj_memory, *, selector=None, need_weights=False, _last_aux=True, _summary_token=None):
+    def readout_query(self, pixel_readout, obj_memory, *, selector=None, need_weights=False, _last_aux=True, _summary_token=None, _defer_out=False):
         assert selector is None, 'selector is a training-time argument'
         eng = self.engine()
+        self.finish_readout()
         px = group_nhwc_of(pixel_readout)
         K, h, w = px.shape[:3]
+        fold = bool(_defer_out) and not _last_aux and plans.eca_fold_ok(eng, self.embed_dim, h * w)
         om = obj_memory[0]
         if om.dtype != F32:
             om = om.to(F32)
@@ -534,13 +537,30 @@
         st = eng.__dict__.setdefault('_qinit_state', {})
         fresh = _summary_token is None or st.get(K) != _summary_token or not plans.QINIT_SKIP
         st[K] = _summary_token
-        P = eng.plan(('rq', K, h, w, bool(_last_aux), fresh), plans.build_readout_query, K, h, w, bool(_last_aux), fresh)
+        P = eng.plan(('rq', K, h, w, bool(_last_aux), fresh, fold), plans.build_readout_query, K, h, w, bool(_last_aux), fresh, 1, fold)
         out = eng.pool.get(('rq', K, h, w, eng.devstr), dict(out=((K, h, w, self.embed_dim), BF16, False)), eng.device)['out']
         P.run(pixel=px, obj_mem=om, out=out)
+        if fold:
+            e = P.meta['eca']
+            eng._eca_pending = (out, P.bufs[e['t2']], P.bufs[e['r']], P.bufs[e['sums']])
         n_aux = P.bufs['aux_logits'].shape[0] - (0 if _last_aux else 1)
         aux = {'logits': [P.bufs['aux_logits'][i].view(1, K, h, w) for i in range(n_aux)],
                'q_weights': None, 'p_weights': None}
         return group_logical(out), aux
+
+    def finish_readout(self):
+        eng = self._eng
+        pend = None if eng is None else eng.__dict__.get('_eca_pending')
+        if pend is None:
+            return
+        eng._eca_pending = None
+        out, t2, r, sums = pend
+        K, h, w, C = out.shape
+        from .. import ops as O
+        ol = O.OpList()
+        nb = self.model_cfg['object_transformer']['num_blocks']
+        ol.eca_apply(t2, None, eng.w[f'object_transformer.blocks.{nb - 1}.pixel_ffn.conv.conv.weight'], r, out, B=K, HW=h * w, C=C, fixed_sums=sums)
+        ol.run()
 
     def segment(self, ms_image_feat: List[torch.Tensor], memory_readout, sensory, *, selector=None, chunk_size=-1,
                 update_sensory=True, _need_logits=True, _fork=False):
@@ -548,6 +568,11 @@
         eng = self.engine()
         dev = eng.device
         p16 = group_nhwc_of(memory_readout)
+        pend = eng.__dict__.get('_eca_pending')
+        fold = pend is not None and p16.data_ptr() == pend[0].data_ptr() and p16.shape == pend[0].shape
+        if pend is not None and not fold:
+            self.finish_readout()
+            p16 = group_nhwc_of(memory_readout)
         K, h, w = p16.shape[:3]
         f8, f4 = nhwc_of(ms_image_feat[1]), nhwc_of(ms_image_feat[2])
         sf, sb = self._sensory_pair(sensory)
@@ -555,7 +580,8 @@
         if pre is not None and pre[2].data_ptr() != f4.data_ptr():
             pre = None
         md = bool(_fork) and K + 1 <= 8 and dev.type == 'cuda'
-        P = eng.plan(('seg', K, h, w, bool(update_sensory), pre is not None, md), plans.build_segment, K, h, w, bool(update_sensory), pre is not None, md)
+        P = eng.plan(('seg', K, h, w, bool(update_sensory), pre is not None, md, fold), plans.build_segment, K, h, w, bool(update_sensory), pre is not None, md,
+                     1, 1, fold)
         sp = dict(prob=((K + 1, 16 * h, 16 * w), F32, False))
         if _need_logits:
             sp['lup'] = ((K + 1, 16 * h, 16 * w), F32, False)
@@ -563,6 +589,9 @@
         prob, lup = o['prob'], o.get('lup')
         feats = dict(f8=f8, f4=f4) if pre is None else dict(f8p=pre[0], f4p=pre[1])
         dyn = dict(p16=p16, sensory_f32=sf, sensory_bf16=sb, prob=prob, logits_up=lup, **feats)
+        if fold:
+            eng._eca_pending = None
+            dyn.update(eca_t2=pend[1], eca_r=pend[2], eca_sums=pend[3])
         n_ops, cut = len(P.ol.recs), P.meta.get('logits_done', 0)
         if _fork and not eng.one_lane and update_sensory and dev.type == 'cuda' and not plans.GRAPHS and 0 < cut < n_ops - 1 and K + 1 <= 16:
             main = torch.cuda.current_stream(dev)
diff --git a/cutie_amd/model/plans.py b/cutie_amd/model/plans.py
--- a/cutie_amd/model/plans.py
+++ b/cutie_amd/model/plans.py
@@ -402,12 +402,18 @@
             c0 = c
         return out
 
-    def ca_block(self, prefix, x, name, out=None, head=None):
+    def ca_block(self, prefix, x, name, out=None, head=None, defer=False):
         if head is not None:
             head = (self.eng.w[head[0]], head[1])
         w = self.eng.w[prefix + '.conv2']
+        HW = x.H * x.W
+        if defer:
+            assert eca_fold_ok(self.eng, x.C, HW) and O.conv_side_jobs_ok(cin=x.C, cout=w.cout, kh=w.kh)
+            sums = self.buf(name + '.gapsum', (x.B, x.C), torch.int64, persistent=True)
+            t1 = self.conv(prefix + '.conv1', x, name=name + '.t1', relu_in=True, act=O.ACT_RELU, zero=sums)
+            self.conv(prefix + '.conv2', t1, name=name + '.t2', gap_acc=sums, persistent=True)
+            return dict(t2=name + '.t2', sums=name + '.gapsum')
         gap = self.buf(name + '.gap', (x.B, x.C), F32)
-        HW = x.H * x.W
         if O.conv_side_jobs_ok(cin=x.C, cout=w.cout, kh=w.kh):
             sums = self.buf(name + '.gapsum', (x.B, x.C), torch.int64)
             t1 = self.conv(prefix + '.conv1', x, name=name + '.t1', relu_in=True, act=O.ACT_RELU, zero=sums)
@@ -465,6 +471,12 @@
         return Dyn(a.t.name, a.t.offset + s0 * per_obj * elem)
     assert a.t.is_contiguous() and a.t.element_size() == elem, (a.t.shape, a.t.dtype, elem)
     return a.t.reshape(-1)[s0 * per_obj:]
+
+
+def eca_fold_ok(eng, C, HW):
+    ex = _lib.get_executor()
+    ex = getattr(ex, 'ex', ex)
+    return (not ex.is_mock and C == 256 and HW >= 2 and O.conv_side_jobs_ok(cin=C, cout=C, kh=3) and _lib.has_eca_fold())
 
 
 MIXED_FUSION_EXTRA = 1
@@ -575,7 +587,8 @@
     return P
 
 
-def build_readout_query(eng, K, h, w, last_aux=True, fresh=True, clips=1):
+def build_readout_query(eng, K, h, w, last_aux=True, fresh=True, clips=1, fold_eca=False):
+    fold_eca = bool(fold_eca) and eca_fold_ok(eng, eng.m['embed_dim'], h * w)
     G, counts, st, mixed = clip_layout(K, clips)
     K = st[-1]
     Kc = counts if mixed else counts[0]
@@ -692,10 +705,13 @@
                 kv2 = f(n + 'kv2', (M, 2 * C))
                 ol.linear(x, W[q + '.read_from_query.kv'], kv2, M=M, x_add=query_emb, add_rows=M, add_cols=C)
                 ol.attn_p2q(kvq.t.view(-1)[2 * C:], kv2, kv2.view(-1)[C:], pa, K=K, Q=Q, HW=HW, C=C, heads=heads, ldq=3 * C, ldkv=2 * C)
-        pf = P.conv(q + '.read_from_query.out', Act(pa, K, h, w, C), name=n + 'pf', res=pixel)
         last = b == nb - 1
+        pf = P.conv(q + '.read_from_query.out', Act(pa, K, h, w, C), name=n + 'pf', res=pixel, persistent=last and fold_eca)
         want_aux = not last or last_aux
         fuse_head = want_aux and C == 256
+        if last and fold_eca:
+            P.meta['eca'] = dict(P.ca_block(q + '.pixel_ffn.conv', pf, n + 'ffn', defer=True), r=n + 'pf', head=want_aux)
+            break
         pixel = P.ca_block(q + '.pixel_ffn.conv', pf, n + 'ffn', out=Act(Dyn('out'), K, h, w, C) if last else None,
                            head=(f'{t}.mask_pred.{b + 1}.1', aux[b + 1]) if fuse_head else None)
         if want_aux and not fuse_head:
@@ -705,10 +721,11 @@
     return P
 
 
-def build_segment(eng, K, h, w, update_sensory, pre=False, md=False, clips=1, wstride=1):
+def build_segment(eng, K, h, w, update_sensory, pre=False, md=False, clips=1, wstride=1, fold_eca=False, eca_head=False):
     G, counts, st, mixed = clip_layout(K, clips)
     K = st[-1]
     Kc = max(counts)
+    assert not fold_eca or eca_fold_ok(eng, eng.m['mask_decoder']['up_dims'][0], h * w)
     assert G == 1 or (pre and Kc + 1 <= 8), 'clips in lock step: image-only decoder convs from the encoder plan, <= 7 objects per clip'
     P = Plan(eng, touch=weights_go_cold(h * w, K))
     P.mixed = counts if mixed else None
@@ -728,7 +745,13 @@
         f4p = P.conv('mask_decoder.decoder_feat_proc.transforms.1', Act(Dyn('f4'), 1, h4, w4, ms[2]), name='f4p')
     p16 = Act(Dyn('p16'), K, h, w, up[0])
     u8 = P.buf('u8', (K, h8, w8, up[0]))
-    ol.upsample2x_add(p16.t, f8p.t, u8, B=K, h=h, w=w, C=up[0], skip_group=(sgrp, wstride * h8 * w8) if G > 1 else None)
+    eca = None
+    if fold_eca:
+        t = 'object_transformer'
+        nb = m[t]['num_blocks']
+        eca = dict(t2=Dyn('eca_t2'), r=Dyn('eca_r'), sums=Dyn('eca_sums'), wk=eng.w[f'{t}.blocks.{nb - 1}.pixel_ffn.conv.conv.weight'],
+                   head=(eng.w[f'{t}.mask_pred.{nb}.1'], Dyn('eca_logits')) if eca_head else None)
+    ol.upsample2x_add(p16.t, f8p.t, u8, B=K, h=h, w=w, C=up[0], skip_group=(sgrp, wstride * h8 * w8) if G > 1 else None, eca=eca)
     u8 = Act(u8, K, h8, w8, up[0])
     t1 = P.conv('mask_decoder.up_16_8.out_conv.conv1', u8, relu_in=True, act=O.ACT_RELU)
     ds = P.conv('mask_decoder.up_16_8.out_conv.downsample', u8)
diff --git a/cutie_amd/ops.py b/cutie_amd/ops.py
--- a/cutie_amd/ops.py
+++ b/cutie_amd/ops.py
@@ -26,6 +26,7 @@
 F_TILE_OFF = 128 if os.environ.get('CUTIE_AMD_COUT1_TILE', '1') in ('', '0') else 0
 ACT_NONE, ACT_RELU, ACT_SIGMOID, ACT_SQ1 = 0, 1, 2, 3
 ACT_SHIFT = 4
+UP2_ECA = 1
 AREA_RT = 8 if os.environ.get('CUTIE_AMD_AREA_R', '1') in ('', '0') else 0
 GRU_SCALAR = 1 if os.environ.get('CUTIE_AMD_GRU4', '1') in ('', '0') else 0
 KEYPREP_LOOP = 2 if os.environ.get('CUTIE_AMD_KEYPREP_LOOP', '0') not in ('', '0') else 0
@@ -435,8 +436,18 @@
     def img_prep(self, image, masks, y, *, h0, w0, H, W, pad_left, pad_top, K, mean, std):
         return self.add(IMG_PREP, 0, [h0, w0, H, W, pad_left, pad_top, K], list(mean) + list(std), [image, masks, y])
 
-    def upsample2x_add(self, g, skip, y, *, B, h, w, C, skip_group=None):
+    def upsample2x_add(self, g, skip, y, *, B, h, w, C, skip_group=None, eca=None):
         ints = [B, h, w, C]
+        if eca is not None:
+            assert C == 256 and h * w >= 2, (C, h, w)
+            tail = [eca['t2'], eca['r'], eca['sums'], eca['wk'], eca.get('gap')]
+            if eca.get('head') is not None:
+                hw_, out = eca['head']
+                assert hw_.cout == 1 and hw_.kh == 1 and hw_.cin_padded == 256
+                tail += [hw_.weight, hw_.bias, out]
+            flags, ptrs = UP2_ECA, [g, skip, y] + tail
+        else:
+            flags, ptrs = 0, [g, skip, y]
         if skip_group is not None and not isinstance(skip_group[0], int):
             counts, stride = skip_group
             assert sum(counts) == B and stride >= 4 * h * w
@@ -445,7 +456,7 @@
             kg, stride = int(skip_group[0]), int(skip_group[1])
             assert kg > 0 and B % kg == 0 and stride >= 4 * h * w
             ints += [kg, stride]
-        return self.add(UPSAMPLE2X_ADD, 0, ints, [], [g, skip, y])
+        return self.add(UPSAMPLE2X_ADD, flags, ints, [], ptrs)
 
     def area_down(self, x, y, *, B, H, W, C, ldx, ldy, r, f32_in=False, Cz=None):
         return self.add(AREA_DOWN, 1 if f32_in else 0, [B, H, W, C, ldx, ldy, r, C if Cz is None else Cz], [], [x, y])
```
